# ProgramerSalar/stable-diffusion-from-scratch

Hardware: AMD Instinct MI355X
Metric: images/sec (512×512, 50-step DDIM) at 1/2/4/8 MI355X; UNet step ms (higher is better)
Workload: dtype f16; 1 GPU; sd1-txt2img-512-ddim50; global_batch=16, batch_per_gpu=16, ddim_steps=50, parallelism=dp1

## Files before the change

include/sdk_amd.h:

```cpp
#ifndef SDK_AMD_H
#define SDK_AMD_H

#include <stdint.h>

#ifdef __cplusplus
extern "C" {
#endif

typedef void* sdk_stream_t;

enum sdk_status {
  SDK_OK = 0,
  SDK_EINVAL = -1,
  SDK_EHIP = -2,
  SDK_EWORKSPACE = -3
};

typedef struct {
  const void* src0;
  const void* src1;
  int32_t c_split;
  int32_t cin;
  int32_t ld0, ld1;
  int32_t h, w;
  int32_t ksize;
  int32_t stride, pad;
  int32_t upsample;
  const float* gn_scale;
  const float* gn_shift;
  int32_t silu;
  int32_t pad_end;
} sdk_conv_src;

enum sdk_out_mode {
  SDK_OUT_NHWC_F16 = 0,
  SDK_OUT_NCHW_F32 = 1,
  SDK_OUT_GEGLU_F16 = 2,
  SDK_OUT_ROWS_F32 = 3
};

typedef struct {
  int32_t batch, ho, wo, cout;
  int32_t nseg;
  sdk_conv_src seg[2];
  const void* weight;
  int32_t k_total;
  const float* bias;
  const float* row_bias;
  int32_t row_bias_ld;
  const void* residual;
  int32_t res_ld;
  void* out;
  int32_t out_ld;
  int32_t out_mode;
  int32_t split_k;
  float* workspace;
  int64_t workspace_bytes;
  int32_t variant_hint;
  int32_t act;
  float* gn_partial;
  int64_t weight_batch_stride;
  int32_t split_inlaunch;
  uint32_t* tile_counters;
  int32_t tile_group_m;
  int32_t upsample_phase;
} sdk_conv_args;

#define SDK_TILE_COUNTERS 16384

enum sdk_conv_act {
  SDK_ACT_NONE = 0,
  SDK_ACT_QUICK_GELU = 1,
  SDK_ACT_GELU = 2
};

typedef struct {
  int32_t split_k;
  int32_t grid_tiles;
  int64_t workspace_bytes;
  int32_t variant;
  double flops;
  int32_t gn_chunks;
} sdk_conv_plan_info;

int sdk_conv2d_plan(const sdk_conv_args* a, sdk_conv_plan_info* info);
int sdk_conv2d(const sdk_conv_args* a, sdk_stream_t stream);

typedef struct {
  const void* src0; const void* src1;
  int32_t c_split, ld0, ld1;
  int32_t batch, hw, channels, groups;
  float eps;
  const float* gamma; const float* beta;
  float* scale; float* shift;
  float* workspace; int64_t workspace_bytes;
} sdk_group_norm_args;

int64_t sdk_group_norm_workspace(int32_t batch, int32_t hw, int32_t channels);
int sdk_group_norm_affine(const sdk_group_norm_args* a, sdk_stream_t stream);

int sdk_group_norm_apply(const sdk_group_norm_args* a, int32_t silu, void* y, int32_t ld_y, sdk_stream_t stream);

int sdk_group_norm_apply_padded(const sdk_group_norm_args* a, int32_t silu, void* y, int32_t ld_y, int32_t h,
                                int32_t w, int32_t pad, sdk_stream_t stream);

int sdk_group_norm(const sdk_group_norm_args* a, int32_t silu, void* y, int32_t ld_y, int32_t h, int32_t w,
                   int32_t pad, const float* part0, int32_t nch0, const float* part1, int32_t nch1,
                   sdk_stream_t stream);

int sdk_group_norm_finalize(const sdk_group_norm_args* a, const float* part0, int32_t nch0, const float* part1,
                            int32_t nch1, sdk_stream_t stream);

int sdk_group_norm_apply_ex(const sdk_group_norm_args* a, int32_t silu, const float* post_bias, int32_t pb_ld,
                            const void* residual, int32_t res_ld, void* y, int32_t ld_y, sdk_stream_t stream);

enum { SDK_GN_STATS_GIVEN = 0,
       SDK_GN_STATS_SLICE,
       SDK_GN_STATS_CHUNKED,
       SDK_GN_STATS_PARTS };
enum { SDK_GN_APPLY_NONE = 0,
       SDK_GN_APPLY_IN_STATS,
       SDK_GN_APPLY_FLAT, SDK_GN_APPLY_ROW, SDK_GN_APPLY_STRIDE };
typedef struct { int32_t stats, apply, launches; int64_t workspace_bytes; } sdk_group_norm_plan_info;
int sdk_group_norm_plan(const sdk_group_norm_args* a, int32_t want_stats, int32_t want_apply, int32_t h, int32_t w,
                        int32_t pad, int32_t nch0, int32_t nch1, int32_t allow_single_launch,
                        sdk_group_norm_plan_info* info);

double sdk_probe_mfma_flops(int32_t m16, int32_t blocks, int32_t iters);
int sdk_probe_mfma(int32_t m16, int32_t blocks, int32_t iters, const void* seed, float* sink, sdk_stream_t stream);
int sdk_probe_copy(const void* src, void* dst, int64_t bytes, sdk_stream_t stream);
int sdk_probe_copy_ex(const void* src, void* dst, int64_t bytes, int32_t mode, sdk_stream_t stream);

int sdk_layer_norm(const void* x, void* y, int32_t rows, int32_t cols, int32_t ld_x, int32_t ld_y,
                   const float* gamma, const float* beta, float eps, sdk_stream_t stream);

typedef struct {
  const void* q; const void* k; const void* v; void* o;
  int32_t q_ld, k_ld, v_ld, o_ld;
  int32_t batch, heads, nq, nk, head_dim;
  float scale;
  int32_t causal;
} sdk_attention_args;

int sdk_attention(const sdk_attention_args* a, sdk_stream_t stream);

enum { SDK_ATTN_AUTO = 0, SDK_ATTN_NW4, SDK_ATTN_NW8, SDK_ATTN_NW8_STAG, SDK_ATTN_QB2, SDK_ATTN_WIDE };
#define SDK_ATTN_WIDE_ROWS 64
#define SDK_ATTN_WIDE_KT 32
typedef struct { int32_t form, dqk, dv, waves, qblocks, stagger, seed_col, causal, grid; } sdk_attention_form_info;
int sdk_attention_form(const sdk_attention_args* a, int32_t form, sdk_attention_form_info* ran ,
                       sdk_stream_t stream);

typedef struct {
  const void* q; const void* k; const void* v; void* o;
  int32_t q_ld, k_ld, v_ld, o_ld;
  int32_t batch, heads, n, dim_head;
  void* workspace; int64_t workspace_bytes;
} sdk_linear_attention_args;
int32_t sdk_linear_attention_chunks(int32_t n);
int64_t sdk_linear_attention_workspace_bytes(const sdk_linear_attention_args* a);
int sdk_linear_attention(const sdk_linear_attention_args* a, sdk_stream_t stream);

typedef struct {
  const void* t; const void* kv; const void* wq; const void* wo; const float* bias; const void* res;
  void* out;
  int32_t t_ld, kv_ld, w_ld, res_ld, out_ld;
  int32_t batch, n_img, nk, channels, head_dim;
  float scale;
} sdk_xattn_args;

int sdk_cross_attention_block_supported(int32_t channels, int32_t head_dim, int32_t nk, int32_t n_img);
int sdk_xattn_pack_weight(const void* w, int32_t w_ld, void* packed, int32_t channels, sdk_stream_t stream);
int sdk_cross_attention_block(const sdk_xattn_args* a, sdk_stream_t stream);

typedef struct {
  const float* in_gamma; const float* in_beta; float in_eps;
  const float* out_gamma; const float* out_beta; float out_eps;
  void* out_ln; int32_t out_ln_ld;
} sdk_xattn_ln_args;

int sdk_cross_attention_block_ln(const sdk_xattn_args* a, const sdk_xattn_ln_args* ln, sdk_stream_t stream);

int sdk_segment_softmax(const float* s, int32_t ld_s, void* p, int32_t ld_p, int32_t rows, int32_t nseg,
                        int32_t seglen, float scale, sdk_stream_t stream);

typedef struct {
  const void* t; const void* res; void* out; const void* packed; const float* b2;
  int32_t t_ld, res_ld, out_ld;
  int32_t rows, channels, features;
} sdk_ff_args;

int sdk_ff_supported(int32_t channels, int32_t features);
int64_t sdk_ff_packed_bytes(int32_t channels, int32_t features);
int sdk_ff_pack(const void* w1, const float* b1, const void* w2, void* packed, int32_t channels, int32_t features,
                sdk_stream_t stream);
int sdk_feed_forward(const sdk_ff_args* a, sdk_stream_t stream);

typedef struct {
  const void* x; const void* w; const float* bias; const void* res; void* out;
  int32_t x_ld, res_ld, out_ld;
  int32_t rows, in_features, out_features;
} sdk_token_linear_args;

int sdk_token_linear_supported(int32_t in_features, int32_t out_features);
int sdk_token_linear(const sdk_token_linear_args* a, sdk_stream_t stream);

int sdk_token_linear_ln(const sdk_token_linear_args* a, const float* gamma, const float* beta, float eps,
                        void* out_ln, int32_t out_ln_ld, sdk_stream_t stream);

typedef struct {
  const float* x; const float* e; const float* e_uncond; const float* noise;
  float* x_prev; float* pred_x0;
  int64_t n;
  float sqrt_one_minus_at, sqrt_at, dir_coef, sqrt_a_prev, sigma, temperature;
  float guidance;
  int32_t v_param;
  float v_sqrt_a, v_sqrt_1ma;
} sdk_ddim_args;

int sdk_ddim_step(const sdk_ddim_args* a, sdk_stream_t stream);

int sdk_ddim_xprev(const sdk_ddim_args* a, sdk_stream_t stream);

typedef struct {
  const float* x; const float* model_out; const float* noise; const float* x_recon_in;
  float* x_prev; float* x_recon;
  int64_t n;
  int32_t stage, x0_param, clip;
  float c_recip, c_recipm1, coef1, coef2, sigma, nonzero, temperature;
} sdk_posterior_args;

int sdk_posterior_step(const sdk_posterior_args* a, sdk_stream_t stream);

typedef struct {
  const float* x0; const float* noise; const float* mask; const float* img;
  float* out;
  int64_t n, per_sample;
  int32_t hw, mask_mode;
  float sqrt_acp, sqrt_1m_acp;
} sdk_masked_q_args;

int sdk_masked_q_sample(const sdk_masked_q_args* a, sdk_stream_t stream);

int sdk_cfg_combine(const float* e_uncond, const float* e_cond, float* out, int64_t n, float guidance,
                    sdk_stream_t stream);

typedef struct {
  sdk_ddim_args step;
  int32_t pred_x0_in;
  float drop_scale;
  const uint8_t* keep;
  sdk_masked_q_args blend;
} sdk_ddim_ex_args;

int sdk_ddim_step_ex(const sdk_ddim_ex_args* a, sdk_stream_t stream);

typedef struct {
  sdk_posterior_args step;
  const uint8_t* keep;
  float drop_scale;
} sdk_posterior_ex_args;

int sdk_posterior_step_ex(const sdk_posterior_ex_args* a, sdk_stream_t stream);

enum { SDK_MULTISTEP_PLMS = 0, SDK_MULTISTEP_PLMS_WARMUP = 1, SDK_MULTISTEP_DPM = 2 };

typedef struct {
  sdk_ddim_args step;
  const float* hist[3];
  const float* e_next;
  float* hist_out;
  int32_t form, nhist;
  float c_x, c_0, c_1;
  int32_t reserved;
  sdk_masked_q_args blend;
} sdk_multistep_args;

int sdk_multistep_step(const sdk_multistep_args* a, sdk_stream_t stream);

typedef struct {
  const float* src[4];
  int32_t channels[4];
  int32_t nsrc;
  void* y;
  int32_t batch, hw, c_pad;
} sdk_concat_args;

int sdk_concat_nchw_to_nhwc(const sdk_concat_args* a, sdk_stream_t stream);

typedef struct {
  const float* src[4];
  int32_t channels[4];
  int32_t nsrc;
  void* y;
  int32_t batch, h, w, c_pad;
  int32_t kh, kw, sy, sx;
  int32_t p0, np;
} sdk_patch_pack_args;

int sdk_patch_pack(const sdk_patch_pack_args* a, sdk_stream_t stream);

int sdk_vq_code_norms(const float* codebook, float* norms, int32_t n, int32_t d, sdk_stream_t stream);

int32_t sdk_vq_nearest_splits(int64_t m, int32_t n, int32_t d);

int sdk_vq_nearest(const float* z, const float* codebook, const float* norms, int64_t* idx, float* z_q,
                   int32_t batch, int32_t d, int32_t hw, int32_t n, void* keys, int64_t keys_bytes,
                   int32_t force_splits, sdk_stream_t stream);

int sdk_vq_lookup(const int64_t* idx, const float* codebook, float* out, int64_t m, int32_t n, int32_t d,
                  int32_t hw, int32_t nchw, sdk_stream_t stream);

int sdk_vq_remap(const int64_t* inds, const int64_t* used, const int64_t* rnd, int64_t* out, int64_t count,
                 int32_t n_used, int32_t mode, int64_t unknown, int32_t extra, sdk_stream_t stream);

int sdk_ddpm_step(const float* x, const float* eps, const float* noise, float* out, int64_t n,
                  float inv_sqrt_alpha, float coef, float sigma, sdk_stream_t stream);

int sdk_timestep_embedding(const int64_t* t, const float* freqs, void* out, int32_t batch, int32_t dim,
                           sdk_stream_t stream);

int sdk_nchw_to_nhwc(const float* x, void* y, int32_t batch, int32_t channels, int32_t hw, int32_t c_pad,
                     float scale, sdk_stream_t stream);

int sdk_diag_gaussian_sample(const float* moments, const float* noise, float* z, int32_t batch, int32_t channels,
                             int32_t hw, float scale, sdk_stream_t stream);

int sdk_stochastic_encode(const float* x0, const float* noise, float* out, int64_t n, float sqrt_a,
                          float sqrt_1ma, sdk_stream_t stream);

int sdk_token_embedding(const int64_t* ids, const float* tok, const float* pos, void* out, int32_t batch,
                        int32_t seq, int32_t dim, sdk_stream_t stream);

int sdk_extract_patches(const float* z, float* out, int32_t batch, int32_t channels, int32_t h, int32_t w,
                        int32_t kh, int32_t kw, int32_t sy, int32_t sx, sdk_stream_t stream);
int sdk_fold_patches(const float* patches, const float* pix_w, const float* l_w, float* out, int32_t batch,
                     int32_t channels, int32_t h, int32_t w, int32_t ph, int32_t pw, int32_t sy, int32_t sx,
                     int32_t ly, int32_t lx, sdk_stream_t stream);

int sdk_upsample_bilinear2x(const void* x, void* y, int32_t batch, int32_t h, int32_t w, int32_t channels,
                            sdk_stream_t stream);
int sdk_gelu(const void* x, void* y, int64_t n, sdk_stream_t stream);

int sdk_upsample_nearest2x_padded(const void* x, int32_t ld_x, void* y, int32_t batch, int32_t h, int32_t w,
                                  int32_t channels, int32_t pad, sdk_stream_t stream);

int sdk_zero_border(const void* x, int32_t ld_x, void* y, int32_t batch, int32_t h, int32_t w, int32_t channels,
                    int32_t pad, sdk_stream_t stream);

int sdk_group_norm_film(const sdk_group_norm_args* a, const float* film, int32_t film_ld, int32_t film_off,
                        int32_t silu, void* y, int32_t ld_y, int32_t h, int32_t w, int32_t pad, const float* part0,
                        int32_t nch0, const float* part1, int32_t nch1, sdk_stream_t stream);

enum { SDK_RESAMPLE_AVGPOOL2 = 0, SDK_RESAMPLE_NEAREST2 = 1 };
int sdk_group_norm_resample(const sdk_group_norm_args* a, int32_t mode, int32_t silu, int32_t h, int32_t w,
                            int32_t pad, void* y_act, void* y_raw, sdk_stream_t stream);

int sdk_embedding_add(const void* emb, const float* table, const int64_t* ids, void* out, int32_t batch, int32_t dim,
                      int32_t n, sdk_stream_t stream);

int sdk_embedding_rows(const int64_t* ids, const float* table, void* out, int32_t n, int32_t dim,
                       sdk_stream_t stream);

enum { SDK_RESIZE_NEAREST = 0, SDK_RESIZE_BILINEAR = 1, SDK_RESIZE_BICUBIC = 2, SDK_RESIZE_AREA = 3 };
typedef struct {
  const float* x;
  float* y;
  int32_t planes, h, w, out_h, out_w, mode;
  double scale_h, scale_w;
} sdk_resize2d_args;

int sdk_resize2d(const sdk_resize2d_args* a, sdk_stream_t stream);

const char* sdk_last_error(void);
int sdk_version(void);
const char* sdk_kernel_name(int32_t variant);

#ifdef __cplusplus
}
#endif
#endif
```

stable-diffusion-from-scratch_amd/_lib.py:

```python
from __future__ import annotations

import ctypes as C
import os

_HERE = os.path.dirname(os.path.abspath(__file__))
LIB_PATH = os.environ.get("SD_AMD_LIB") or os.path.join(_HERE, "libsdk_amd.so")

vp = C.c_void_p
i32 = C.c_int32
i64 = C.c_int64
f32 = C.c_float
fp = C.POINTER(C.c_float)


class ConvSrc(C.Structure):
    _fields_ = [("src0", vp), ("src1", vp), ("c_split", i32), ("cin", i32), ("ld0", i32), ("ld1", i32),
                ("h", i32), ("w", i32), ("ksize", i32), ("stride", i32), ("pad", i32), ("upsample", i32),
                ("gn_scale", vp), ("gn_shift", vp), ("silu", i32), ("pad_end", i32)]


class ConvArgs(C.Structure):
    _fields_ = [("batch", i32), ("ho", i32), ("wo", i32), ("cout", i32), ("nseg", i32), ("seg", ConvSrc * 2),
                ("weight", vp), ("k_total", i32), ("bias", vp), ("row_bias", vp), ("row_bias_ld", i32),
                ("residual", vp), ("res_ld", i32), ("out", vp), ("out_ld", i32), ("out_mode", i32),
                ("split_k", i32), ("workspace", vp), ("workspace_bytes", i64), ("variant_hint", i32),
                ("act", i32), ("gn_partial", vp), ("weight_batch_stride", i64), ("split_inlaunch", i32),
                ("tile_counters", vp), ("tile_group_m", i32), ("upsample_phase", i32)]


class ConvPlanInfo(C.Structure):
    _fields_ = [("split_k", i32), ("grid_tiles", i32), ("workspace_bytes", i64), ("variant", i32),
                ("flops", C.c_double), ("gn_chunks", i32)]


class GroupNormArgs(C.Structure):
    _fields_ = [("src0", vp), ("src1", vp), ("c_split", i32), ("ld0", i32), ("ld1", i32), ("batch", i32),
                ("hw", i32), ("channels", i32), ("groups", i32), ("eps", f32), ("gamma", vp), ("beta", vp),
                ("scale", vp), ("shift", vp), ("workspace", vp), ("workspace_bytes", i64)]


class GroupNormPlanInfo(C.Structure):
    _fields_ = [("stats", i32), ("apply", i32), ("launches", i32), ("workspace_bytes", i64)]


class AttentionArgs(C.Structure):
    _fields_ = [("q", vp), ("k", vp), ("v", vp), ("o", vp), ("q_ld", i32), ("k_ld", i32), ("v_ld", i32),
                ("o_ld", i32), ("batch", i32), ("heads", i32), ("nq", i32), ("nk", i32), ("head_dim", i32),
                ("scale", f32), ("causal", i32)]


class AttentionFormInfo(C.Structure):
    _fields_ = [("form", i32), ("dqk", i32), ("dv", i32), ("waves", i32), ("qblocks", i32), ("stagger", i32),
                ("seed_col", i32), ("causal", i32), ("grid", i32)]


class LinearAttentionArgs(C.Structure):
    _fields_ = [("q", vp), ("k", vp), ("v", vp), ("o", vp), ("q_ld", i32), ("k_ld", i32), ("v_ld", i32),
                ("o_ld", i32), ("batch", i32), ("heads", i32), ("n", i32), ("dim_head", i32), ("workspace", vp),
                ("workspace_bytes", i64)]


class XAttnArgs(C.Structure):
    _fields_ = [("t", vp), ("kv", vp), ("wq", vp), ("wo", vp), ("bias", vp), ("res", vp), ("out", vp),
                ("t_ld", i32), ("kv_ld", i32), ("w_ld", i32), ("res_ld", i32), ("out_ld", i32), ("batch", i32),
                ("n_img", i32), ("nk", i32), ("channels", i32), ("head_dim", i32), ("scale", f32)]


class XAttnLnArgs(C.Structure):
    _fields_ = [("in_gamma", vp), ("in_beta", vp), ("in_eps", f32), ("out_gamma", vp), ("out_beta", vp),
                ("out_eps", f32), ("out_ln", vp), ("out_ln_ld", i32)]


class FfArgs(C.Structure):
    _fields_ = [("t", vp), ("res", vp), ("out", vp), ("packed", vp), ("b2", vp), ("t_ld", i32), ("res_ld", i32),
                ("out_ld", i32), ("rows", i32), ("channels", i32), ("features", i32)]


class TokenLinearArgs(C.Structure):
    _fields_ = [("x", vp), ("w", vp), ("bias", vp), ("res", vp), ("out", vp), ("x_ld", i32), ("res_ld", i32),
                ("out_ld", i32), ("rows", i32), ("in_features", i32), ("out_features", i32)]


class DdimArgs(C.Structure):
    _fields_ = [("x", vp), ("e", vp), ("e_uncond", vp), ("noise", vp), ("x_prev", vp), ("pred_x0", vp),
                ("n", i64), ("sqrt_one_minus_at", f32), ("sqrt_at", f32), ("dir_coef", f32), ("sqrt_a_prev", f32),
                ("sigma", f32), ("temperature", f32), ("guidance", f32), ("v_param", i32), ("v_sqrt_a", f32),
                ("v_sqrt_1ma", f32)]


class PosteriorArgs(C.Structure):
    _fields_ = [("x", vp), ("model_out", vp), ("noise", vp), ("x_recon_in", vp), ("x_prev", vp), ("x_recon", vp),
                ("n", i64), ("stage", i32), ("x0_param", i32), ("clip", i32), ("c_recip", f32), ("c_recipm1", f32),
                ("coef1", f32), ("coef2", f32), ("sigma", f32), ("nonzero", f32), ("temperature", f32)]


class MaskedQArgs(C.Structure):
    _fields_ = [("x0", vp), ("noise", vp), ("mask", vp), ("img", vp), ("out", vp), ("n", i64), ("per_sample", i64),
                ("hw", i32), ("mask_mode", i32), ("sqrt_acp", f32), ("sqrt_1m_acp", f32)]


class DdimExArgs(C.Structure):
    _fields_ = [("step", DdimArgs), ("pred_x0_in", i32), ("drop_scale", f32), ("keep", vp), ("blend", MaskedQArgs)]


class MultistepArgs(C.Structure):
    _fields_ = [("step", DdimArgs), ("hist", vp * 3), ("e_next", vp), ("hist_out", vp), ("form", i32), ("nhist", i32),
                ("c_x", f32), ("c_0", f32), ("c_1", f32), ("reserved", i32), ("blend", MaskedQArgs)]


class PosteriorExArgs(C.Structure):
    _fields_ = [("step", PosteriorArgs), ("keep", vp), ("drop_scale", f32)]


class ConcatArgs(C.Structure):
    _fields_ = [("src", vp * 4), ("channels", i32 * 4), ("nsrc", i32), ("y", vp), ("batch", i32), ("hw", i32),
                ("c_pad", i32)]


class PatchPackArgs(C.Structure):
    _fields_ = [("src", vp * 4), ("channels", i32 * 4), ("nsrc", i32), ("y", vp), ("batch", i32), ("h", i32),
                ("w", i32), ("c_pad", i32), ("kh", i32), ("kw", i32), ("sy", i32), ("sx", i32), ("p0", i32),
                ("np", i32)]


class Resize2dArgs(C.Structure):
    _fields_ = [("x", vp), ("y", vp), ("planes", i32), ("h", i32), ("w", i32), ("out_h", i32), ("out_w", i32),
                ("mode", i32), ("scale_h", C.c_double), ("scale_w", C.c_double)]


OUT_NHWC_F16, OUT_NCHW_F32, OUT_GEGLU_F16, OUT_ROWS_F32 = 0, 1, 2, 3
RESIZE_NEAREST, RESIZE_BILINEAR, RESIZE_BICUBIC, RESIZE_AREA = range(4)
ACT_NONE, ACT_QUICK_GELU, ACT_GELU = 0, 1, 2
ATTN_AUTO, ATTN_NW4, ATTN_NW8, ATTN_NW8_STAG, ATTN_QB2, ATTN_WIDE = range(6)
MULTISTEP_PLMS, MULTISTEP_PLMS_WARMUP, MULTISTEP_DPM = range(3)
ATTN_WIDE_ROWS, ATTN_WIDE_KT = 64, 32
RESAMPLE_AVGPOOL2, RESAMPLE_NEAREST2 = 0, 1
GN_STATS = ("given", "slice", "chunked", "parts")
GN_APPLY = ("none", "in_stats", "flat", "row", "stride")

EXPORTS = ["sdk_conv2d_plan", "sdk_conv2d", "sdk_group_norm_workspace", "sdk_group_norm_affine", "sdk_group_norm_apply", "sdk_group_norm_apply_padded", "sdk_group_norm_apply_ex", "sdk_group_norm", "sdk_group_norm_finalize", "sdk_group_norm_plan", "sdk_layer_norm",
           "sdk_attention", "sdk_attention_form", "sdk_linear_attention", "sdk_linear_attention_workspace_bytes", "sdk_linear_attention_chunks", "sdk_cross_attention_block_supported", "sdk_xattn_pack_weight", "sdk_cross_attention_block", "sdk_cross_attention_block_ln", "sdk_segment_softmax", "sdk_ff_supported", "sdk_ff_packed_bytes", "sdk_ff_pack", "sdk_feed_forward", "sdk_token_linear_supported", "sdk_token_linear", "sdk_token_linear_ln", "sdk_ddim_step", "sdk_ddim_xprev", "sdk_ddim_step_ex", "sdk_multistep_step", "sdk_cfg_combine", "sdk_posterior_step", "sdk_posterior_step_ex", "sdk_masked_q_sample", "sdk_concat_nchw_to_nhwc", "sdk_patch_pack", "sdk_ddpm_step", "sdk_timestep_embedding", "sdk_nchw_to_nhwc",
           "sdk_diag_gaussian_sample", "sdk_stochastic_encode", "sdk_token_embedding", "sdk_extract_patches",
           "sdk_fold_patches", "sdk_vq_code_norms", "sdk_vq_nearest_splits", "sdk_vq_nearest", "sdk_vq_lookup", "sdk_vq_remap",
           "sdk_upsample_bilinear2x", "sdk_upsample_nearest2x_padded", "sdk_zero_border", "sdk_gelu",
           "sdk_group_norm_film", "sdk_group_norm_resample", "sdk_embedding_add", "sdk_embedding_rows", "sdk_resize2d", "sdk_last_error", "sdk_version", "sdk_kernel_name",
           "sdk_probe_mfma_flops", "sdk_probe_mfma", "sdk_probe_copy", "sdk_probe_copy_ex"]

_lib = None


def lib():
    global _lib
    if _lib is not None:
        return _lib
    if not os.path.exists(LIB_PATH):
        raise RuntimeError(f"sd_amd: HIP library not built ({LIB_PATH} missing); run __graft_entry__.build()")
    import torch
    L = C.CDLL(LIB_PATH)
    L.sdk_conv2d_plan.argtypes = [C.POINTER(ConvArgs), C.POINTER(ConvPlanInfo)]
    L.sdk_conv2d.argtypes = [C.POINTER(ConvArgs), vp]
    L.sdk_group_norm_workspace.argtypes = [i32, i32, i32]
    L.sdk_group_norm_workspace.restype = i64
    L.sdk_group_norm_affine.argtypes = [C.POINTER(GroupNormArgs), vp]
    L.sdk_group_norm_apply.argtypes = [C.POINTER(GroupNormArgs), i32, vp, i32, vp]
    L.sdk_group_norm_apply_padded.argtypes = [C.POINTER(GroupNormArgs), i32, vp, i32, i32, i32, i32, vp]
    L.sdk_group_norm_apply_ex.argtypes = [C.POINTER(GroupNormArgs), i32, vp, i32, vp, i32, vp, i32, vp]
    L.sdk_group_norm.argtypes = [C.POINTER(GroupNormArgs), i32, vp, i32, i32, i32, i32, vp, i32, vp, i32, vp]
    L.sdk_group_norm_finalize.argtypes = [C.POINTER(GroupNormArgs), vp, i32, vp, i32, vp]
    L.sdk_group_norm_film.argtypes = [C.POINTER(GroupNormArgs), vp, i32, i32, i32, vp, i32, i32, i32, i32, vp, i32, vp,
                                      i32, vp]
    L.sdk_group_norm_plan.argtypes = [C.POINTER(GroupNormArgs), i32, i32, i32, i32, i32, i32, i32, i32,
                                      C.POINTER(GroupNormPlanInfo)]
    L.sdk_group_norm_resample.argtypes = [C.POINTER(GroupNormArgs), i32, i32, i32, i32, i32, vp, vp, vp]
    L.sdk_embedding_add.argtypes = [vp, vp, vp, vp, i32, i32, i32, vp]
    L.sdk_embedding_rows.argtypes = [vp, vp, vp, i32, i32, vp]
    L.sdk_resize2d.argtypes = [C.POINTER(Resize2dArgs), vp]
    L.sdk_upsample_bilinear2x.argtypes = [vp, vp, i32, i32, i32, i32, vp]
    L.sdk_upsample_nearest2x_padded.argtypes = [vp, i32, vp, i32, i32, i32, i32, i32, vp]
    L.sdk_zero_border.argtypes = [vp, i32, vp, i32, i32, i32, i32, i32, vp]
    L.sdk_gelu.argtypes = [vp, vp, i64, vp]
    L.sdk_layer_norm.argtypes = [vp, vp, i32, i32, i32, i32, vp, vp, f32, vp]
    L.sdk_attention.argtypes = [C.POINTER(AttentionArgs), vp]
    L.sdk_attention_form.argtypes = [C.POINTER(AttentionArgs), i32, C.POINTER(AttentionFormInfo), vp]
    L.sdk_linear_attention.argtypes = [C.POINTER(LinearAttentionArgs), vp]
    L.sdk_linear_attention_workspace_bytes.argtypes = [C.POINTER(LinearAttentionArgs)]
    L.sdk_linear_attention_workspace_bytes.restype = i64
    L.sdk_linear_attention_chunks.argtypes = [i32]
    L.sdk_linear_attention_chunks.restype = i32
    L.sdk_cross_attention_block_supported.argtypes = [i32, i32, i32, i32]
    L.sdk_xattn_pack_weight.argtypes = [vp, i32, vp, i32, vp]
    L.sdk_cross_attention_block.argtypes = [C.POINTER(XAttnArgs), vp]
    L.sdk_cross_attention_block_ln.argtypes = [C.POINTER(XAttnArgs), C.POINTER(XAttnLnArgs), vp]
    L.sdk_segment_softmax.argtypes = [vp, i32, vp, i32, i32, i32, i32, f32, vp]
    L.sdk_ff_supported.argtypes = [i32, i32]
    L.sdk_ff_packed_bytes.argtypes = [i32, i32]
    L.sdk_ff_packed_bytes.restype = i64
    L.sdk_ff_pack.argtypes = [vp, vp, vp, vp, i32, i32, vp]
    L.sdk_feed_forward.argtypes = [C.POINTER(FfArgs), vp]
    L.sdk_token_linear_supported.argtypes = [i32, i32]
    L.sdk_token_linear.argtypes = [C.POINTER(TokenLinearArgs), vp]
    L.sdk_token_linear_ln.argtypes = [C.POINTER(TokenLinearArgs), vp, vp, f32, vp, i32, vp]
    L.sdk_ddim_step.argtypes = [C.POINTER(DdimArgs), vp]
    L.sdk_ddim_xprev.argtypes = [C.POINTER(DdimArgs), vp]
    L.sdk_posterior_step.argtypes = [C.POINTER(PosteriorArgs), vp]
    L.sdk_ddim_step_ex.argtypes = [C.POINTER(DdimExArgs), vp]
    L.sdk_multistep_step.argtypes = [C.POINTER(MultistepArgs), vp]
    L.sdk_cfg_combine.argtypes = [vp, vp, vp, i64, f32, vp]
    L.sdk_posterior_step_ex.argtypes = [C.POINTER(PosteriorExArgs), vp]
    L.sdk_masked_q_sample.argtypes = [C.POINTER(MaskedQArgs), vp]
    L.sdk_concat_nchw_to_nhwc.argtypes = [C.POINTER(ConcatArgs), vp]
    L.sdk_patch_pack.argtypes = [C.POINTER(PatchPackArgs), vp]
    L.sdk_vq_code_norms.argtypes = [vp, vp, i32, i32, vp]
    L.sdk_vq_nearest_splits.argtypes = [i64, i32, i32]
    L.sdk_vq_nearest_splits.restype = i32
    L.sdk_vq_nearest.argtypes = [vp, vp, vp, vp, vp, i32, i32, i32, i32, vp, i64, i32, vp]
    L.sdk_vq_lookup.argtypes = [vp, vp, vp, i64, i32, i32, i32, i32, vp]
    L.sdk_vq_remap.argtypes = [vp, vp, vp, vp, i64, i32, i32, i64, i32, vp]
    L.sdk_ddpm_step.argtypes = [vp, vp, vp, vp, i64, f32, f32, f32, vp]
    L.sdk_timestep_embedding.argtypes = [vp, vp, vp, i32, i32, vp]
    L.sdk_nchw_to_nhwc.argtypes = [vp, vp, i32, i32, i32, i32, f32, vp]
    L.sdk_diag_gaussian_sample.argtypes = [vp, vp, vp, i32, i32, i32, f32, vp]
    L.sdk_stochastic_encode.argtypes = [vp, vp, vp, i64, f32, f32, vp]
    L.sdk_token_embedding.argtypes = [vp, vp, vp, vp, i32, i32, i32, vp]
    L.sdk_extract_patches.argtypes = [vp, vp, i32, i32, i32, i32, i32, i32, i32, i32, vp]
    L.sdk_fold_patches.argtypes = [vp, vp, vp, vp, i32, i32, i32, i32, i32, i32, i32, i32, i32, i32, vp]
    L.sdk_probe_mfma_flops.argtypes = [i32, i32, i32]
    L.sdk_probe_mfma_flops.restype = C.c_double
    L.sdk_probe_mfma.argtypes = [i32, i32, i32, vp, vp, vp]
    L.sdk_probe_copy.argtypes = [vp, vp, i64, vp]
    L.sdk_probe_copy_ex.argtypes = [vp, vp, i64, i32, vp]
    L.sdk_last_error.restype = C.c_char_p
    L.sdk_kernel_name.restype = C.c_char_p
    L.sdk_kernel_name.argtypes = [i32]
    for name in EXPORTS:
        if not hasattr(L, name):
            raise RuntimeError(f"sd_amd: {LIB_PATH} does not export {name}")
    _lib = L
    return L


def check(rc: int, what: str):
    if rc != 0:
        msg = lib().sdk_last_error().decode(errors="replace")
        raise RuntimeError(f"sd_amd.{what} failed ({rc}): {msg}")
```

stable-diffusion-from-scratch_amd/build.py:

```python
from __future__ import annotations

import concurrent.futures as cf
import os
import re
import subprocess

HERE = os.path.dirname(os.path.abspath(__file__))
CSRC = os.path.join(HERE, "csrc")
BUILD = os.path.join(HERE, "build")
LIB = os.path.join(HERE, "libsdk_amd.so")
SOURCES = ["norm.hip", "attention.hip", "attention_wide.hip", "linattn.hip", "sampler.hip", "xattn.hip", "ff.hip", "token.hip", "vq.hip", "cond.hip", "probe.hip"]
CONV_TILE_PARTS = 5


def _units():
    yield "conv_plan.hip", "conv_plan", []
    yield "conv_small.hip", "conv_small", []
    yield "conv_rowpanel.hip", "conv_rowpanel", []
    for k in range(1, CONV_TILE_PARTS + 1):
        yield "conv_tile.hip", f"conv_tile_p{k}", [f"-DSDK_CONV_PART={k}"]
    for src in SOURCES:
        yield src, src.replace(".hip", ""), []


def _deps(src: str, csrc: str):
    headers = [os.path.join(csrc, "common.h"), os.path.join(HERE, "..", "include", "sdk_amd.h")]
    if src.startswith("conv"):
        headers += sorted(os.path.join(csrc, f) for f in os.listdir(csrc) if f.startswith("conv") and f.endswith(".h"))
    return [os.path.join(csrc, src)] + headers
HIPCC = os.environ.get("HIPCC", "/opt/rocm/bin/hipcc")
FLAGS = ["--offload-arch=gfx950", "-O3", "-fPIC", "-std=c++17", "-Wno-unused-result"]
EXTRA = {"attention.hip": ["-mno-amdgpu-ieee", "-fno-honor-nans"],
         "attention_wide.hip": ["-mno-amdgpu-ieee", "-fno-honor-nans"]}
REMARK = "-Rpass-analysis=kernel-resource-usage"
NO_SCRATCH = re.compile(r"token_linear320_kernel|attn_wide_kernel|conv_rowpanel_kernel")
WARN_SCRATCH = re.compile(r"conv_glds_kernel|conv_ph_kernel|ff_geglu_kernel|xattn_block_kernel|attn_fwd_kernel|vq_nearest_")
_RES = re.compile(r"remark: (?:Function Name: (\S+)|\s+(VGPRs|AGPRs|ScratchSize \[bytes/lane\]|Occupancy \[waves/SIMD\]): (\d+))")


def resource_usage(stderr: str):
    out = []
    for m in _RES.finditer(stderr):
        if m.group(1):
            out.append((m.group(1), {}))
        elif out:
            out[-1][1][m.group(2).split(" ")[0]] = int(m.group(3))
    return out


def _needs(obj: str, deps) -> bool:
    if not os.path.exists(obj):
        return True
    t = os.path.getmtime(obj)
    return any(os.path.getmtime(d) > t for d in deps)


def build(force: bool = False, verbose: bool = False, diag: bool = False, tag: str = "", defines=(),
          extra=None, csrc: str = CSRC) -> str:
    suffix = "_diag" if diag else (f"_{tag}" if tag else "")
    bdir = BUILD + suffix
    lib = LIB.replace(".so", f"{suffix}.so")
    extra_flags = dict(EXTRA)
    for k, v in (extra or {}).items():
        extra_flags[k] = extra_flags.get(k, []) + list(v)
    os.makedirs(bdir, exist_ok=True)
    jobs = []
    objs = []
    for src, stem, udefs in _units():
        s = os.path.join(csrc, src)
        o = os.path.join(bdir, stem + ".o")
        objs.append(o)
        flags_file = o + ".flags"
        dflags = (["-DSDK_CONV_DIAGNOSTICS"] if diag else []) + list(defines) + udefs
        fl = " ".join(FLAGS + extra_flags.get(src, []) + dflags)
        stale_flags = not os.path.exists(flags_file) or open(flags_file).read() != fl
        if force or stale_flags or _needs(o, _deps(src, csrc)) or not os.path.exists(o + ".res"):
            for stale in (o, flags_file):
                if os.path.exists(stale):
                    os.remove(stale)
            jobs.append(([HIPCC, *FLAGS, *dflags, *extra_flags.get(src, []), REMARK, "-c", s, "-o", o],
                         (flags_file, fl)))

    def run(cmd, sidecar=None):
        r = subprocess.run(cmd, capture_output=True, text=True)
        if r.returncode != 0:
            raise RuntimeError(f"hipcc failed: {' '.join(cmd)}\n{r.stdout}\n{r.stderr}")
        if REMARK in cmd:
            usage = resource_usage(r.stderr)
            obj = cmd[cmd.index("-o") + 1]
            with open(obj + ".res", "w") as f:
                for name, u in usage:
                    f.write(f"{name} vgpr={u.get('VGPRs')} agpr={u.get('AGPRs')} scratch={u.get('ScratchSize')} "
                            f"occ={u.get('Occupancy')}\n")
            if os.path.basename(obj).startswith("token") and not any(
                    NO_SCRATCH.search(n) and "ScratchSize" in u for n, u in usage):
                os.remove(obj)
                raise RuntimeError("no kernel-resource-usage remark for token_linear320_kernel: cannot verify "
                                   "that it uses no scratch")
            bad = [n for n, u in usage if NO_SCRATCH.search(n) and u.get("ScratchSize", 0) > 0]
            for n, u in usage:
                if WARN_SCRATCH.search(n) and u.get("ScratchSize", 0) > 0:
                    print(f"warning: {n} uses {u['ScratchSize']} B/lane of scratch", flush=True)
            if bad:
                os.remove(obj)
                raise RuntimeError("counted-vmcnt kernels use scratch (spills break the hand-counted waits): " +
                                   ", ".join(bad))
        if sidecar:
            with open(sidecar[0], "w") as f:
                f.write(sidecar[1])
        if verbose:
            print(" ".join(cmd))
        return r

    workers = int(os.environ.get("SD_AMD_BUILD_JOBS", "8"))
    with cf.ThreadPoolExecutor(max_workers=min(workers, max(1, len(jobs)))) as ex:
        list(ex.map(lambda j: run(*j), jobs))
    if force or jobs or _needs(lib, objs):
        run([HIPCC, "--offload-arch=gfx950", "-shared", "-fPIC", *objs, "-o", lib])
        with open(os.path.join(bdir, "resource_usage.txt"), "w") as f:
            for o in objs:
                if os.path.exists(o + ".res"):
                    f.write(open(o + ".res").read())
    return lib


if __name__ == "__main__":
    import sys
    print(build(verbose=True, diag="--diag" in sys.argv))
```

stable-diffusion-from-scratch_amd/csrc/common.h:

```cpp
#pragma once
#include <hip/hip_runtime.h>
#include <stdint.h>

#include <atomic>
#include <string>

#include "../../include/sdk_amd.h"

namespace sdk {

typedef _Float16 half_t;
typedef _Float16 h8 __attribute__((ext_vector_type(8)));
typedef _Float16 h4 __attribute__((ext_vector_type(4)));
typedef _Float16 h2 __attribute__((ext_vector_type(2)));
typedef float f16v __attribute__((ext_vector_type(16)));
typedef float f4 __attribute__((ext_vector_type(4)));
typedef float f2 __attribute__((ext_vector_type(2)));

void set_error(const std::string& msg);
int fail(int code, const std::string& msg);
int check_launch(const char* what);
int attention_wide(const sdk_attention_args* a, hipStream_t s, sdk_attention_form_info* ran);

inline int ensure_dyn_lds(const void* fn, int bytes, std::atomic<unsigned long long>& done, const char* what) {
  int dev = 0;
  if (hipGetDevice(&dev) != hipSuccess) return fail(SDK_EHIP, std::string(what) + ": hipGetDevice failed");
  const unsigned long long bit = 1ull << (dev & 63);
  if (done.load(std::memory_order_acquire) & bit) return SDK_OK;
  if (hipFuncSetAttribute(fn, hipFuncAttributeMaxDynamicSharedMemorySize, bytes) != hipSuccess)
    return fail(SDK_EHIP, std::string(what) + ": cannot raise the dynamic LDS limit");
  done.fetch_or(bit, std::memory_order_acq_rel);
  return SDK_OK;
}

__device__ __forceinline__ float silu_f(float x) { return x / (1.0f + __expf(-x)); }
__device__ __forceinline__ float erf_fast(float x) {
  const float a = fabsf(x);
  const float t = __builtin_amdgcn_rcpf(fmaf(0.3275911f, a, 1.0f));
  float y = fmaf(1.061405429f, t, -1.453152027f);
  y = fmaf(y, t, 1.421413741f);
  y = fmaf(y, t, -0.284496736f);
  y = fmaf(y, t, 0.254829592f);
  y *= t;
  const float r = 1.0f - y * __expf(-a * a);
  return copysignf(r, x);
}
__device__ __forceinline__ float gelu_erf(float x) { return 0.5f * x * (1.0f + erf_fast(x * 0.70710678118654752f)); }

__device__ __forceinline__ int xcd_remap(int bid, int nblk) {
  const int q = nblk >> 3, r = nblk & 7, x = bid & 7, i = bid >> 3;
  return (x < r ? x * (q + 1) : r * (q + 1) + (x - r) * q) + i;
}

#ifndef SDK_XLANE_DPP
#define SDK_XLANE_DPP 0
#endif
template <int CTRL>
__device__ __forceinline__ float dpp_f(float x) {
  static_assert(CTRL <= 0xFF || CTRL == 0x124 || CTRL == 0x128, "dpp_f: quad_perm, row_ror:4 or row_ror:8");
#if SDK_XLANE_DPP
  return __builtin_bit_cast(float, __builtin_amdgcn_update_dpp(0, __builtin_bit_cast(int, x), CTRL, 0xF, 0xF, false));
#else
  constexpr int pat = CTRL <= 0xFF ? 0x8000 | CTRL : (0x1F | ((CTRL == 0x124 ? 4 : 8) << 10));
  return __builtin_bit_cast(float, __builtin_amdgcn_ds_swizzle(__builtin_bit_cast(int, x), pat));
#endif
}
__device__ __forceinline__ float readlane_f(float x, int l) {
  return __builtin_bit_cast(float, __builtin_amdgcn_readlane(__builtin_bit_cast(int, x), l));
}
__device__ __forceinline__ float wave_sum_f(float x) {
  x += dpp_f<0xB1>(x);
  x += dpp_f<0x4E>(x);
  x += dpp_f<0x124>(x);
  x += dpp_f<0x128>(x);
  return (readlane_f(x, 0) + readlane_f(x, 16)) + (readlane_f(x, 32) + readlane_f(x, 48));
}

template <int MAXV>
__device__ __forceinline__ void ln_row_stats(const h8 (&v)[MAXV], int cols, float eps, float& mean, float& rstd) {
#pragma clang fp contract(off)
  const int lane = threadIdx.x & 63;
  const int c8 = cols / 8;
  const float x0 = readlane_f((float)v[0][0], 0);
  float s1 = 0.f, s2 = 0.f;
#pragma unroll
  for (int i = 0; i < MAXV; ++i) {
    const bool ok = lane + 64 * i < c8;
#pragma unroll
    for (int j = 0; j < 8; ++j) {
      const float d = ok ? (float)v[i][j] - x0 : 0.f;
      s1 += d;
      s2 = __builtin_fmaf(d, d, s2);
    }
  }
  s1 = wave_sum_f(s1);
  s2 = wave_sum_f(s2);
  const float inv_n = 1.f / cols;
  const float dm = s1 * inv_n;
  const float var = fmaxf(__builtin_fmaf(-dm, dm, s2 * inv_n), 0.f);
  mean = x0 + dm;
  rstd = rsqrtf(var + eps);
}

template <int CPL>
__device__ __forceinline__ void ln_quad_stats(const h8 (&v)[CPL], float eps, float& mean, float& rstd) {
#pragma clang fp contract(off)
  const float x0 = dpp_f<0x00>((float)v[0][0]);
  float s1 = 0.f, s2 = 0.f;
#pragma unroll
  for (int i = 0; i < CPL; ++i)
#pragma unroll
    for (int j = 0; j < 8; ++j) {
      const float d = (float)v[i][j] - x0;
      s1 += d;
      s2 = __builtin_fmaf(d, d, s2);
    }
  s1 += dpp_f<0xB1>(s1);
  s2 += dpp_f<0xB1>(s2);
  s1 += dpp_f<0x4E>(s1);
  s2 += dpp_f<0x4E>(s2);
  const float inv_n = 1.f / (32 * CPL);
  const float dm = s1 * inv_n;
  const float var = fmaxf(__builtin_fmaf(-dm, dm, s2 * inv_n), 0.f);
  mean = x0 + dm;
  rstd = rsqrtf(var + eps);
}

__device__ __forceinline__ h8 ln_quad_apply(const h8& v, float mean, float rstd, const float* gb, int C, int k) {
#pragma clang fp contract(off)
  const f4 g0 = *reinterpret_cast<const f4*>(gb + 8 * k), g1 = *reinterpret_cast<const f4*>(gb + 8 * k + 4);
  const f4 b0 = *reinterpret_cast<const f4*>(gb + C + 8 * k), b1 = *reinterpret_cast<const f4*>(gb + C + 8 * k + 4);
  h8 o;
#pragma unroll
  for (int j = 0; j < 4; ++j) {
    o[j] = (half_t)__builtin_fmaf(((float)v[j] - mean) * rstd, g0[j], b0[j]);
    o[4 + j] = (half_t)__builtin_fmaf(((float)v[4 + j] - mean) * rstd, g1[j], b1[j]);
  }
  return o;
}

__device__ __forceinline__ h8 ln_apply8(const h8& v, float mean, float rstd, const float (&g)[8], const float (&b)[8]) {
#pragma clang fp contract(off)
  h8 o;
#pragma unroll
  for (int j = 0; j < 8; ++j) o[j] = (half_t)__builtin_fmaf(((float)v[j] - mean) * rstd, g[j], b[j]);
  return o;
}

}
```

stable-diffusion-from-scratch_amd/csrc/norm.hip:

```cpp
#include <algorithm>
#include <string>

#include "common.h"

namespace sdk {
namespace {

constexpr int GN_U = 8;

struct GnGeom {
  int c8, nv, ry, chunk_rows, nchunks;
};

GnGeom gn_geom(int batch, int hw, int channels) {
  GnGeom g;
  g.c8 = channels / 8;
  g.nv = (g.c8 + 255) / 256;
  g.ry = g.nv > 1 ? 1 : std::max(1, 256 / g.c8);
  const int step = g.ry * GN_U;
  const int want = std::max(1, (1536 + batch - 1) / std::max(batch, 1));
  const int per = std::max(1, (hw + want - 1) / want);
  g.chunk_rows = (per + step - 1) / step * step;
  g.nchunks = (hw + g.chunk_rows - 1) / g.chunk_rows;
  return g;
}

__device__ __forceinline__ h8 load_px(const half_t* s0, const half_t* s1, int c_split, int ld0, int ld1,
                                      size_t pix, int c) {
  if (c < c_split) return *reinterpret_cast<const h8*>(s0 + pix * ld0 + c);
  return *reinterpret_cast<const h8*>(s1 + pix * ld1 + (c - c_split));
}

__device__ __forceinline__ void gn_load8(const float* p, float o[8]) {
  const f4* q = reinterpret_cast<const f4*>(p);
  const f4 a = q[0], b = q[1];
#pragma unroll
  for (int j = 0; j < 4; ++j) { o[j] = a[j]; o[4 + j] = b[j]; }
}

__device__ __forceinline__ float gn_act(float x, float sc, float sh, int silu) {
  float t = x * sc + sh;
  if (silu) t = t * __builtin_amdgcn_rcpf(1.0f + __expf(-t));
  return t;
}

__device__ __forceinline__ h8 gn_act8(h8 v, const float sc[8], const float sh[8], int silu) {
  h8 o;
#pragma unroll
  for (int j = 0; j < 8; ++j) o[j] = (half_t)gn_act((float)v[j], sc[j], sh[j], silu);
  return o;
}

__global__ void __launch_bounds__(256) gn_partial_kernel(const half_t* s0, const half_t* s1, int c_split, int ld0,
                                                         int ld1, int hw, int channels, GnGeom g, float2* partial) {
  extern __shared__ __attribute__((aligned(16))) float red[];
  const int tid = threadIdx.x, chunk = blockIdx.x, b = blockIdx.y;
  const int r0 = chunk * g.chunk_rows, r1 = min(hw, r0 + g.chunk_rows);
  const size_t img = (size_t)b * hw;
  const int ysub = tid / g.c8;
  for (int vi = 0; vi < g.nv; ++vi) {
    const int vec = g.nv > 1 ? tid + vi * 256 : tid % g.c8;
    const bool active = vec < g.c8 && ysub < g.ry;
    float sum[8], sq[8], piv[8];
#pragma unroll
    for (int j = 0; j < 8; ++j) { sum[j] = 0.f; sq[j] = 0.f; piv[j] = 0.f; }
    if (active) {
      const int c = vec * 8;
      const h8 pv = load_px(s0, s1, c_split, ld0, ld1, img, c);
#pragma unroll
      for (int j = 0; j < 8; ++j) piv[j] = (float)pv[j];
      const int rstart = r0 + (g.nv > 1 ? 0 : ysub);
      const int rstep = g.nv > 1 ? 1 : g.ry;
      for (int r = rstart; r < r1; r += GN_U * rstep) {
        h8 v[GN_U];
#pragma unroll
        for (int u = 0; u < GN_U; ++u) {
          const int rr = r + u * rstep;
          v[u] = rr < r1 ? load_px(s0, s1, c_split, ld0, ld1, img + rr, c) : pv;
        }
#pragma unroll
        for (int u = 0; u < GN_U; ++u)
#pragma unroll
          for (int j = 0; j < 8; ++j) {
            const float d = (float)v[u][j] - piv[j];
            sum[j] += d;
            sq[j] += d * d;
          }
      }
    }
    if (g.ry == 1) {
      if (active) {
#pragma unroll
        for (int j = 0; j < 8; ++j)
          partial[((size_t)b * g.nchunks + chunk) * channels + vec * 8 + j] = make_float2(sum[j], sq[j]);
      }
      continue;
    }
    const int C = g.c8 * 8;
    if (active) {
#pragma unroll
      for (int j = 0; j < 8; ++j) {
        red[ysub * C + vec * 8 + j] = sum[j];
        red[(g.ry + ysub) * C + vec * 8 + j] = sq[j];
      }
    }
    __syncthreads();
    for (int c = tid; c < C; c += 256) {
      float a = 0.f, q = 0.f;
      for (int y = 0; y < g.ry; ++y) { a += red[y * C + c]; q += red[(g.ry + y) * C + c]; }
      partial[((size_t)b * g.nchunks + chunk) * channels + c] = make_float2(a, q);
    }
  }
}

__device__ __forceinline__ double wave_sum_d(double v) {
  for (int off = 32; off > 0; off >>= 1) v += __shfl_xor(v, off, 64);
  return v;
}

__global__ void __launch_bounds__(256) gn_finalize_kernel(const half_t* s0, const half_t* s1, int c_split, int ld0,
                                                          int ld1, int hw, int channels, int groups, GnGeom g,
                                                          const float2* partial, float eps, const float* gamma,
                                                          const float* beta, float* scale, float* shift) {
  __shared__ double cm[256], cq[256];
  const int grp = blockIdx.x, b = blockIdx.y, tid = threadIdx.x, lane = tid & 63, wave = tid >> 6;
  const int cg = channels / groups, c0 = grp * cg;
  const size_t img = (size_t)b * hw;
  const double n = (double)hw;
  int tpc = 64;
  while (tpc > 1 && tpc * cg > 256) tpc >>= 1;
  const int ci = tid / tpc, sub = tid - ci * tpc;
  for (int cbase = 0; cbase < cg; cbase += 256 / tpc) {
    const int cc = cbase + ci;
    const bool act = ci < 256 / tpc && cc < cg;
    double a1 = 0.0, a2 = 0.0;
    if (act) {
      const float2* pp = partial + (size_t)b * g.nchunks * channels + c0 + cc;
      for (int k = sub; k < g.nchunks; k += tpc) {
        const float2 v = pp[(size_t)k * channels];
        a1 += v.x;
        a2 += v.y;
      }
    }
    for (int off = tpc >> 1; off > 0; off >>= 1) {
      a1 += __shfl_xor(a1, off, 64);
      a2 += __shfl_xor(a2, off, 64);
    }
    if (act && sub == 0) {
      const int c = c0 + cc;
      const float piv = c < c_split ? (float)s0[img * ld0 + c] : (float)s1[img * ld1 + (c - c_split)];
      cm[cc] = (double)piv + a1 / n;
      cq[cc] = a2 - a1 * a1 / n;
    }
  }
  __syncthreads();
  if (wave != 0) return;
  double mean_sum = 0.0, m2_sum = 0.0, msq_sum = 0.0;
  for (int ci = lane; ci < cg; ci += 64) {
    mean_sum += cm[ci];
    msq_sum += cm[ci] * cm[ci];
    m2_sum += cq[ci];
  }
  mean_sum = wave_sum_d(mean_sum);
  msq_sum = wave_sum_d(msq_sum);
  m2_sum = wave_sum_d(m2_sum);
  const double mg = mean_sum / cg;
  double m2g = m2_sum + n * (msq_sum - cg * mg * mg);
  if (m2g < 0) m2g = 0;
  const double var = m2g / (n * cg);
  const float rstd = (float)(1.0 / sqrt(var + (double)eps));
  const float meanf = (float)mg;
  for (int ci = lane; ci < cg; ci += 64) {
    const int c = c0 + ci;
    const float gm = gamma ? gamma[c] : 1.f, bt = beta ? beta[c] : 0.f;
    const float sc = gm * rstd;
    scale[(size_t)b * channels + c] = sc;
    shift[(size_t)b * channels + c] = bt - meanf * sc;
  }
}

constexpr int GNF_T = 512;
template <bool APPLY>
__global__ void __launch_bounds__(GNF_T) gn_stats_fused_kernel(const half_t* s0, const half_t* s1, int c_split,
                                                               int ld0, int ld1, int hw, int channels, int cg,
                                                               int gps, float eps, const float* gamma,
                                                               const float* beta, float* scale, float* shift,
                                                               int silu, half_t* y, int ldy, int h, int w, int pad) {
  __shared__ float2 red[GNF_T * 8];
  __shared__ double cmean[512], cm2[512];
  const int tid = threadIdx.x, b = blockIdx.y;
  const int sc = gps * cg, c0 = blockIdx.x * sc;
  const int cv = sc / 8, rp = GNF_T / cv;
  const int v = tid % cv, r0 = tid / cv;
  const bool active = r0 < rp;
  const size_t img = (size_t)b * hw;
  const int c = c0 + 8 * v;
  float sum[8], sq[8], piv[8];
#pragma unroll
  for (int j = 0; j < 8; ++j) { sum[j] = 0.f; sq[j] = 0.f; piv[j] = 0.f; }
  if (active) {
    const h8 pv = load_px(s0, s1, c_split, ld0, ld1, img, c);
#pragma unroll
    for (int j = 0; j < 8; ++j) piv[j] = (float)pv[j];
    constexpr int U = 8;
    for (int r = r0; r < hw; r += U * rp) {
      h8 x[U];
#pragma unroll
      for (int u = 0; u < U; ++u) {
        const int rr = r + u * rp;
        x[u] = rr < hw ? load_px(s0, s1, c_split, ld0, ld1, img + rr, c) : pv;
      }
#pragma unroll
      for (int u = 0; u < U; ++u)
#pragma unroll
        for (int j = 0; j < 8; ++j) {
          const float d = (float)x[u][j] - piv[j];
          sum[j] += d;
          sq[j] += d * d;
        }
    }
#pragma unroll
    for (int j = 0; j < 8; ++j) red[r0 * sc + 8 * v + j] = make_float2(sum[j], sq[j]);
  }
  __syncthreads();
  const double n = (double)hw;
  for (int k = tid; k < sc; k += GNF_T) {
    double a1 = 0.0, a2 = 0.0;
    for (int r = 0; r < rp; ++r) {
      const float2 q = red[r * sc + k];
      a1 += q.x;
      a2 += q.y;
    }
    const int cc = c0 + k;
    const float p0 = cc < c_split ? (float)s0[img * ld0 + cc] : (float)s1[img * ld1 + (cc - c_split)];
    cmean[k] = (double)p0 + a1 / n;
    cm2[k] = a2 - a1 * a1 / n;
  }
  __syncthreads();
  for (int g = tid; g < gps; g += GNF_T) {
    double ms = 0.0, m2 = 0.0;
    for (int k = 0; k < cg; ++k) ms += cmean[g * cg + k];
    const double mg = ms / cg;
    for (int k = 0; k < cg; ++k) {
      const double dm = cmean[g * cg + k] - mg;
      m2 += cm2[g * cg + k] + n * dm * dm;
    }
    const double var = (m2 > 0 ? m2 : 0.0) / (n * cg);
    cmean[g * cg] = mg;
    cm2[g * cg] = 1.0 / sqrt(var + (double)eps);
  }
  __syncthreads();
  for (int k = tid; k < sc; k += GNF_T) {
    const int g = k / cg, cc = c0 + k;
    const float rstd = (float)cm2[g * cg], meanf = (float)cmean[g * cg];
    const float gm = gamma ? gamma[cc] : 1.f, bt = beta ? beta[cc] : 0.f;
    const float s = gm * rstd;
    if constexpr (APPLY) {
      red[k] = make_float2(s, bt - meanf * s);
    } else {
      scale[(size_t)b * channels + cc] = s;
      shift[(size_t)b * channels + cc] = bt - meanf * s;
    }
  }
  if constexpr (APPLY) {
    __syncthreads();
    if (!active) return;
    float sa[8], sh[8];
#pragma unroll
    for (int j = 0; j < 8; ++j) {
      const float2 t = red[8 * v + j];
      sa[j] = t.x;
      sh[j] = t.y;
    }
    const int wp = w + 2 * pad, npix = (h + 2 * pad) * wp;
    half_t* yb = y + (size_t)b * npix * ldy + c;
    constexpr int U = 4;
    for (int r = r0; r < npix; r += U * rp) {
      h8 x[U];
      bool in[U];
#pragma unroll
      for (int u = 0; u < U; ++u) {
        const int rr = r + u * rp;
        const int py = rr / wp - pad, px = rr - (rr / wp) * wp - pad;
        in[u] = rr < npix && (unsigned)py < (unsigned)h && (unsigned)px < (unsigned)w;
        x[u] = in[u] ? load_px(s0, s1, c_split, ld0, ld1, img + (size_t)py * w + px, c) : h8{};
      }
#pragma unroll
      for (int u = 0; u < U; ++u) {
        const int rr = r + u * rp;
        if (rr >= npix) continue;
        h8 o = {};
        if (in[u]) o = gn_act8(x[u], sa, sh, silu);
        *reinterpret_cast<h8*>(yb + (size_t)rr * ldy) = o;
      }
    }
  }
}

template <class Put>
__device__ __forceinline__ void gn_merge_group(const double* cm, const double* cq, int cg, double n, float eps, int c0,
                                               const float* gamma, const float* beta, int lane, Put put) {
  double mean_sum = 0.0;
  for (int ci = lane; ci < cg; ci += 64) mean_sum += cm[ci];
  mean_sum = wave_sum_d(mean_sum);
  const double mg = mean_sum / cg;
  double m2g = 0.0;
  for (int ci = lane; ci < cg; ci += 64) {
    const double dm = cm[ci] - mg;
    m2g += cq[ci] + n * dm * dm;
  }
  m2g = wave_sum_d(m2g);
  const double var = (m2g > 0 ? m2g : 0.0) / (n * cg);
  const float rstd = (float)(1.0 / sqrt(var + (double)eps));
  const float meanf = (float)mg;
  for (int ci = lane; ci < cg; ci += 64) {
    const int c = c0 + ci;
    const float gm = gamma ? gamma[c] : 1.f, bt = beta ? beta[c] : 0.f;
    const float sc = gm * rstd;
    put(ci, c, sc, bt - meanf * sc);
  }
}

__global__ void __launch_bounds__(256) gn_finalize_part_kernel(const float2* part0, int nch0, const float2* part1,
                                                               int nch1, int c_split, int hw, int channels,
                                                               int groups, float eps, const float* gamma,
                                                               const float* beta, float* scale, float* shift) {
  __shared__ double cm[256], cq[256];
  const int grp = blockIdx.x, b = blockIdx.y, tid = threadIdx.x, lane = tid & 63, wave = tid >> 6;
  const int cg = channels / groups, c0 = grp * cg;
  int tpc = 64;
  while (tpc > 1 && tpc * cg > 256) tpc >>= 1;
  const int ci = tid / tpc, sub = tid - ci * tpc;
  for (int cbase = 0; cbase < cg; cbase += 256 / tpc) {
    const int cc = cbase + ci;
    const bool act = ci < 256 / tpc && cc < cg;
    double mean = 0.0, m2 = 0.0, n = 0.0;
    if (act) {
      const int c = c0 + cc;
      const bool second = c >= c_split;
      const float2* pp = second ? part1 : part0;
      const int nch = second ? nch1 : nch0, cs = second ? channels - c_split : c_split, cl = second ? c - c_split : c;
      const double rows = (double)hw / nch;
      for (int k = sub; k < nch; k += tpc) {
        const float2 q = pp[((size_t)b * nch + k) * cs + cl];
        const double dl = (double)q.x - mean, nn = n + rows, f = rows / nn;
        mean += dl * f;
// ... 907 lines not shown
```

stable-diffusion-from-scratch_amd/openai_model/attention.py:

```python
from __future__ import annotations

import os
import math

import torch
from torch import nn

from .. import ops
from ..packing import f32, gn_norm, prep_norm
from .utils import conv_nd, normalization, zero_module


def Normalize(in_channels):
    return torch.nn.GroupNorm(num_groups=32, num_channels=in_channels, eps=1e-6, affine=True)


_FUSED_ENV = os.environ.get("SD_AMD_FUSED_XATTN")
FUSED_CROSS_ATTENTION = _FUSED_ENV != "0"
FUSED_XATTN_MIN_ROWS = 0 if _FUSED_ENV == "1" else 65536
FUSED_XATTN_640_MAX_ROWS = 16384
FUSED_XATTN_NORMS = os.environ.get("SD_AMD_XATTN_NORMS") != "0"


def _use_fused_xattn(channels, head_dim, nk, n_img, batch):
    if not FUSED_CROSS_ATTENTION or n_img % 64:
        return False
    rows = batch * n_img
    if _FUSED_ENV != "1":
        if channels == 320:
            if rows < FUSED_XATTN_MIN_ROWS:
                return False
        elif channels != 640 or rows > FUSED_XATTN_640_MAX_ROWS:
            return False
    return ops.cross_attention_block_supported(channels, head_dim, nk, n_img)


XATTN_REASSOC = os.environ.get("SD_AMD_XATTN_REASSOC") != "0"

FUSED_FF = os.environ.get("SD_AMD_FUSED_FF") != "0"
TOKEN_LINEAR = os.environ.get("SD_AMD_TOKEN_LINEAR", "1") != "0"


class ReassocContext:
    __slots__ = ("kv", "w1", "w2", "heads", "nk", "batch", "_build")

    def __init__(self, kv, heads, nk, batch, build):
        self.kv, self.heads, self.nk, self.batch, self._build = kv, heads, nk, batch, build
        self.w1 = self.w2 = None

    def weights(self):
        if self.w1 is None:
            if torch.cuda.is_available() and torch.cuda.is_current_stream_capturing():
                raise RuntimeError("ReassocContext: per-prompt weights are built eagerly — run one eager "
                                   "step with this context before capturing a graph")
            self.w1, self.w2 = self._build()
            self._build = None
        return self.w1, self.w2


def reassoc_weights(k, v, wq, wo):
    B, L, H, d = k.shape
    w1 = torch.einsum("bjhe,hec->bhjc", k, wq.view(H, d, -1)).reshape(B, H * L, -1)
    w2 = torch.einsum("che,bjhe->bchj", wo.view(wo.shape[0], H, d), v).reshape(B, wo.shape[0], H * L)
    return w1, w2


def _reassoc_applies(inner, heads, nk):
    kr = (heads * nk + ops.BK - 1) // ops.BK * ops.BK
    return XATTN_REASSOC and 2 * kr <= inner


class CrossAttention(nn.Module):

    def __init__(self, query_dim, context_dim=None, heads=8, dim_head=64, dropout=0.):
        super().__init__()
        inner_dim = dim_head * heads
        self.self_attn = context_dim is None
        context_dim = query_dim if context_dim is None else context_dim
        self.scale = dim_head ** -0.5
        self.heads = heads
        self.dim_head = dim_head
        self.to_q = nn.Linear(query_dim, inner_dim, bias=False)
        self.to_k = nn.Linear(context_dim, inner_dim, bias=False)
        self.to_v = nn.Linear(context_dim, inner_dim, bias=False)
        self.to_out = nn.Sequential(nn.Linear(inner_dim, query_dim), nn.Dropout(dropout))

    def _prepare(self, dev):
        qd = self.to_q.in_features
        cd = self.to_k.in_features
        if self.self_attn:
            w = torch.cat([self.to_q.weight, self.to_k.weight, self.to_v.weight], 0)
            self._pc_qkv = ops.PackedConv([(w, qd)], None, device=dev)
        self._pc_q = ops.PackedConv([(self.to_q.weight, qd)], None, device=dev)
        self._pc_kv = ops.PackedConv([(torch.cat([self.to_k.weight, self.to_v.weight], 0), cd)], None, device=dev)
        self._pc_o = ops.PackedConv([(self.to_out[0].weight, self.heads * self.dim_head)], self.to_out[0].bias,
                                    device=dev)
        inner = self.heads * self.dim_head
        self._ptl_o = (ops.PackedTokenLinear(self.to_out[0].weight, self.to_out[0].bias, dev)
                       if self.self_attn and ops.token_linear_supported(inner, self.to_out[0].out_features) else None)
        if not self.self_attn:
            self._bo32 = f32(self.to_out[0].bias, dev)
            self._pc_reassoc = None

    def context_kv(self, ctx2d, L=None):
        kv = ops.linear(self._pc_kv, ctx2d)
        inner = self.heads * self.dim_head
        if L is None or self.self_attn or not _reassoc_applies(inner, self.heads, L):
            return kv
        B, H, d = ctx2d.shape[0] // L, self.heads, self.dim_head
        C = self.to_q.in_features
        Co = self.to_out[0].out_features

        def build():
            dev = kv.device
            if self._pc_reassoc is None:
                wq, wo = self.to_q.weight.detach(), self.to_out[0].weight.detach()
                self._pc_reassoc = (
                    [ops.PackedConv([(wq[h * d:(h + 1) * d].t().contiguous(), d)], None, device=dev) for h in range(H)],
                    [ops.PackedConv([(wo[:, h * d:(h + 1) * d].contiguous(), d)], None, device=dev) for h in range(H)])
            pq, po = self._pc_reassoc
            kr = (H * L + ops.BK - 1) // ops.BK * ops.BK
            w1 = torch.zeros(B, (kr + ops.BN - 1) // ops.BN * ops.BN, C, dtype=torch.float16, device=dev)
            w2 = torch.zeros(B, (Co + ops.BN - 1) // ops.BN * ops.BN, kr, dtype=torch.float16, device=dev)
            w1h = w1[:, :H * L].view(B, H, L, C)
            for h in range(H):
                w1h[:, h] = ops.linear(pq[h], kv[:, h * d:(h + 1) * d]).view(B, L, C)
                w2[:, :Co, h * L:(h + 1) * L] = ops.linear(po[h], kv[:, inner + h * d:inner + (h + 1) * d]).view(
                    B, L, Co).transpose(1, 2)
            return ops.PerImageWeights(w1, H * L), ops.PerImageWeights(w2, Co, self._bo32)
        return ReassocContext(kv, H, L, B, build)

    def _run(self, t, residual, B, N, kv=None, Lc=None):
        inner = self.heads * self.dim_head
        if kv is None:
            if self.self_attn:
                qkv = ops.linear(self._pc_qkv, t)
                q, k, v, nk = qkv[:, :inner], qkv[:, inner:2 * inner], qkv[:, 2 * inner:], N
            else:
                q = ops.linear(self._pc_q, t)
                kvx = ops.linear(self._pc_kv, t)
                k, v, nk = kvx[:, :inner], kvx[:, inner:], N
        else:
            ops.PROFILER.region = "cross_attention"
            if isinstance(kv, ReassocContext):
                if t.stride(-1) == 1 and N % 128 == 0 and kv.batch == B:
                    w1, w2 = kv.weights()
                    s = ops.linear(w1, t, out_mode=ops.OUT_ROWS_F32, n_img=N)
                    p = ops.segment_softmax(s, kv.heads, kv.nk, self.scale, ld_p=w2.k_total)
                    out = ops.linear(w2, p, residual=residual, n_img=N)
                    ops.PROFILER.region = None
                    return out
                kv = kv.kv
            if t.stride(-1) == 1 and _use_fused_xattn(inner, self.dim_head, Lc, N, B):
                out = ops.cross_attention_block(t, kv, self._pc_q, self._pc_o, batch=B, n_img=N, nk=Lc,
                                                heads=self.heads, head_dim=self.dim_head, scale=self.scale,
                                                residual=residual)
                ops.PROFILER.region = None
                return out
            q = ops.linear(self._pc_q, t)
            k, v, nk = kv[:, :inner], kv[:, inner:], Lc
        o = ops.attention(q, k, v, batch=B, heads=self.heads, nq=N, nk=nk, head_dim=self.dim_head, scale=self.scale)
        if TOKEN_LINEAR and self._ptl_o is not None and o.stride(-1) == 1 and \
                (residual is None or residual.is_contiguous()):
            out = ops.token_linear(self._ptl_o, o, residual=residual)
        else:
            out = ops.linear(self._pc_o, o, residual=residual)
        ops.PROFILER.region = None
        return out


class GELU(nn.Module):

    def __init__(self, dim_in, dim_out):
        super().__init__()
        self.proj = nn.Linear(dim_in, dim_out * 2)


class FeedForward(nn.Module):

    def __init__(self, dim, dim_out=None, mult=4, glu=False, dropout=0.):
        super().__init__()
        inner_dim = int(dim * mult)
        dim_out = dim if dim_out is None else dim_out
        if not glu:
            raise NotImplementedError("sd_amd: only the gated (GEGLU) feed-forward is on the SD path")
        self.net = nn.Sequential(GELU(dim, inner_dim), nn.Dropout(dropout), nn.Linear(inner_dim, dim_out))

    def _prepare(self, dev):
        p = self.net[0].proj
        self._pc1 = ops.PackedConv([(p.weight, p.in_features)], p.bias, geglu=True, device=dev)
        self._pc2 = ops.PackedConv([(self.net[2].weight, self.net[2].in_features)], self.net[2].bias, device=dev)
        self._pff = None
        if FUSED_FF and ops.ff_supported(p.in_features, p.out_features // 2):
            self._pff = ops.PackedFF(p.weight, p.bias, self.net[2].weight, self.net[2].bias, dev)

    def _run(self, t, residual):
        if self._pff is not None and t.stride(-1) == 1:
            return ops.feed_forward(self._pff, t, residual=residual)
        g = ops.linear(self._pc1, t, out_mode=ops.OUT_GEGLU_F16)
        return ops.linear(self._pc2, g, residual=residual)


class BasicTransformerBlock(nn.Module):

    def __init__(self, dim, n_heads, d_head, dropout=0., context_dim=None, gated_ff=True, checkpoint=True):
        super().__init__()
        self.attn1 = CrossAttention(query_dim=dim, heads=n_heads, dim_head=d_head, dropout=dropout)
        self.ff = FeedForward(dim=dim, dropout=dropout, glu=gated_ff)
        self.attn2 = CrossAttention(query_dim=dim, context_dim=context_dim, heads=n_heads, dim_head=d_head,
                                    dropout=dropout)
        self.norm1 = nn.LayerNorm(dim)
        self.norm2 = nn.LayerNorm(dim)
        self.norm3 = nn.LayerNorm(dim)
        self.checkpoint = checkpoint

    def _prepare(self, dev):
        for m in (self.attn1, self.attn2, self.ff):
            m._prepare(dev)
        for n in (self.norm1, self.norm2, self.norm3):
            prep_norm(n, dev)

    def _run(self, tok, B, N, kv=None, Lc=None, t=None):
        if t is None:
            t = ops.layer_norm(tok, self.norm1._g, self.norm1._b, self.norm1.eps)
        tok = self.attn1._run(t, tok, B, N)
        a2 = self.attn2
        if (kv is not None and FUSED_XATTN_NORMS and tok.stride(-1) == 1
                and _use_fused_xattn(a2.heads * a2.dim_head, a2.dim_head, Lc, N, B)):
            ops.PROFILER.region = "cross_attention"
            tok, t = ops.cross_attention_block(
                tok, kv, a2._pc_q, a2._pc_o, batch=B, n_img=N, nk=Lc, heads=a2.heads, head_dim=a2.dim_head,
                scale=a2.scale, residual=tok, norm_in=(self.norm2._g, self.norm2._b, self.norm2.eps),
                norm_out=(self.norm3._g, self.norm3._b, self.norm3.eps))
            ops.PROFILER.region = None
            return self.ff._run(t, tok)
        t = ops.layer_norm(tok, self.norm2._g, self.norm2._b, self.norm2.eps)
        tok = self.attn2._run(t, tok, B, N, kv, Lc)
        t = ops.layer_norm(tok, self.norm3._g, self.norm3._b, self.norm3.eps)
        return self.ff._run(t, tok)


class SpatialTransformer(nn.Module):

    def __init__(self, in_channels, n_heads, d_head, depth=1, dropout=0., context_dim=None, use_linear=False):
        super().__init__()
        self.in_channels = in_channels
        inner_dim = n_heads * d_head
        self.inner_dim = inner_dim
        self.use_linear = use_linear
        self.norm = Normalize(in_channels)
        if use_linear:
            self.proj_in = nn.Linear(in_channels, inner_dim)
        else:
            self.proj_in = nn.Conv2d(in_channels, inner_dim, kernel_size=1, stride=1, padding=0)
        self.transformer_blocks = nn.ModuleList(
            [BasicTransformerBlock(inner_dim, n_heads, d_head, dropout=dropout, context_dim=context_dim)
             for _ in range(depth)])
        if use_linear:
            self.proj_out = zero_module(nn.Linear(in_channels, inner_dim))
        else:
            self.proj_out = zero_module(nn.Conv2d(inner_dim, in_channels, kernel_size=1, stride=1, padding=0))

    def _prepare(self, dev):
        prep_norm(self.norm, dev)
        self._pc_in = ops.PackedConv([(self.proj_in.weight, self.in_channels)], self.proj_in.bias, device=dev)
        self._ptl_in = (ops.PackedTokenLinear(self.proj_in.weight, self.proj_in.bias, dev)
                        if ops.token_linear_supported(self.in_channels, self.inner_dim) else None)
        self._pc_out = ops.PackedConv([(self.proj_out.weight, self.inner_dim)], self.proj_out.bias, device=dev)
        for blk in self.transformer_blocks:
            blk._prepare(dev)

    def context_kv(self, ctx2d, L=None):
        return [blk.attn2.context_kv(ctx2d, L) for blk in self.transformer_blocks]

    def _run(self, x, kvs=None, Lc=None):
        B, H, W, Cc = x.shape
        xn = gn_norm(self.norm, x, silu=False)
        t1 = None
        if TOKEN_LINEAR and self._ptl_in is not None and xn.is_contiguous():
            n1 = self.transformer_blocks[0].norm1 if len(self.transformer_blocks) else None
            if n1 is not None:
                tok, t1 = ops.token_linear(self._ptl_in, xn.view(B * H * W, Cc), norm=(n1._g, n1._b, n1.eps))
            else:
                tok = ops.token_linear(self._ptl_in, xn.view(B * H * W, Cc))
        else:
            tok = ops.conv2d(self._pc_in, xn).view(B * H * W, self.inner_dim)
        for i, blk in enumerate(self.transformer_blocks):
            tok = blk._run(tok, B, H * W, None if kvs is None else kvs[i], Lc, t=t1 if i == 0 else None)
        return ops.conv2d(self._pc_out, tok.view(B, H, W, self.inner_dim), residual=x, gn_stats=True)


class QKVAttentionLegacy(nn.Module):

    def __init__(self, n_heads):
        super().__init__()
        self.n_heads = n_heads

    def scale(self, ch):
        return 1.0 / math.sqrt(math.sqrt(ch))


class FlashAttention(nn.Module):

    def __init__(self, n_heads):
        super().__init__()
        self.n_heads = n_heads

    def scale(self, ch):
        return 1.0 / math.sqrt(ch)


class AttentionBlock(nn.Module):

    def __init__(self, channels, num_heads=1, num_head_channels=-1, use_checkpoint=False,
                 use_new_attention_order=False):
        super().__init__()
        self.channels = channels
        if num_head_channels == -1:
            self.num_heads = num_heads
        else:
            assert channels % num_head_channels == 0
            self.num_heads = channels // num_head_channels
        self.use_checkpoint = use_checkpoint
        self.norm = normalization(channels)
        self.qkv = conv_nd(1, channels, channels * 3, 1)
        self.attention = FlashAttention(self.num_heads) if use_new_attention_order else \
            QKVAttentionLegacy(self.num_heads)
        self.proj_out = zero_module(conv_nd(1, channels, channels, 1))

    def _prepare(self, dev):
        self.norm._prepare(dev)
        self._pc_qkv = ops.PackedConv([(self.qkv.weight, self.channels)], self.qkv.bias, device=dev)
        self._pc_proj = ops.PackedConv([(self.proj_out.weight, self.channels)], self.proj_out.bias, device=dev)

    def _run(self, x):
        B, H, W, Cc = x.shape
        xn = self.norm.norm(x, silu=False)
        qkv = ops.conv2d(self._pc_qkv, xn).view(B * H * W, 3 * Cc)
        ch = Cc // self.num_heads
        o = ops.attention(qkv[:, :Cc], qkv[:, Cc:2 * Cc], qkv[:, 2 * Cc:], batch=B, heads=self.num_heads,
                          nq=H * W, nk=H * W, head_dim=ch, scale=self.attention.scale(ch))
        return ops.conv2d(self._pc_proj, o.view(B, H, W, Cc), residual=x, gn_stats=True)
```

stable-diffusion-from-scratch_amd/ops.py:

```python
from __future__ import annotations

import ctypes as C
import math

import numpy as np
import torch

from . import _lib
from ._lib import (ACT_NONE, ACT_QUICK_GELU, ACT_GELU, AttentionArgs, XAttnArgs, XAttnLnArgs, FfArgs, TokenLinearArgs, ConvArgs, ConvPlanInfo, GroupNormArgs,
                   OUT_GEGLU_F16, OUT_NCHW_F32, OUT_NHWC_F16, OUT_ROWS_F32, check, lib)

BK = 64
BN = 128


def _stream():
    return C.c_void_p(torch.cuda.current_stream().cuda_stream)


def _ptr(t):
    return C.c_void_p(t.data_ptr()) if t is not None else None


def _need_cuda(t: torch.Tensor, what: str, dtype=torch.float16):
    if not isinstance(t, torch.Tensor) or not t.is_cuda:
        raise TypeError(f"sd_amd.{what}: expected a CUDA tensor (HIP path only, no CPU fallback)")
    if dtype is not None and t.dtype != dtype:
        raise TypeError(f"sd_amd.{what}: expected {dtype}, got {t.dtype}")


def need_gpu_sampler(option: str, device):
    if torch.device(device).type != "cuda":
        raise NotImplementedError(f"sd_amd: {option} is implemented on the GPU only (HIP kernels, no CPU "
                                  f"fallback); got device '{device}'")



class _Workspace:

    def __init__(self):
        self.buf = {}
        self.retired = []
        self.lane = 0

    def release_retired(self):
        self.retired.clear()

    def use_lane(self, lane: int):
        import contextlib

        @contextlib.contextmanager
        def cm():
            prev, self.lane = self.lane, lane
            try:
                yield
            finally:
                self.lane = prev
        return cm()

    def counters(self, device) -> torch.Tensor:
        key = (torch.device(device).index, self.lane, "cnt")
        c = self.buf.get(key)
        if c is None:
            if torch.cuda.is_current_stream_capturing():
                raise RuntimeError("sd_amd: tile counters must exist before graph capture (run one warm-up step)")
            c = torch.zeros(TILE_COUNTERS, dtype=torch.int32, device=device)
            self.buf[key] = c
        return c

    def get(self, nbytes: int, device) -> torch.Tensor:
        key = (torch.device(device).index, self.lane)
        b = self.buf.get(key)
        if b is None or b.numel() < nbytes:
            if torch.cuda.is_current_stream_capturing():
                raise RuntimeError("sd_amd: workspace must be sized before graph capture (run one warm-up step)")
            if b is not None:
                self.retired.append(b)
                nbytes = max(nbytes, 2 * b.numel())
            b = torch.empty(max(nbytes, 1 << 20), dtype=torch.uint8, device=device)
            self.buf[key] = b
        return b


WORKSPACE = _Workspace()
TILE_COUNTERS = 16384



def _as_pair(x):
    if isinstance(x, tuple):
        a, b = x
        return a, b
    return x, None


def src_shape(x):
    a, b = _as_pair(x)
    B, H, W, C0 = a.shape
    return B, H, W, C0 + (b.shape[-1] if b is not None else 0)


def _fill_src(s: "_lib.ConvSrc", x, ksize, stride, pad, upsample, gn, silu):
    a, b = _as_pair(x)
    _need_cuda(a, "conv2d")
    B, H, W, C0 = a.shape
    if a.stride(3) != 1 or (H > 1 and a.stride(1) != W * a.stride(2)) or (B > 1 and a.stride(0) != H * a.stride(1)):
        raise ValueError("sd_amd.conv2d: source must be NHWC with contiguous channels and a uniform pixel stride")
    s.src0 = a.data_ptr()
    s.ld0 = a.stride(2) if a.dim() == 4 else a.stride(1)
    if b is not None:
        _need_cuda(b, "conv2d")
        s.src1 = b.data_ptr()
        s.ld1 = b.stride(2)
        s.c_split = C0
        s.cin = C0 + b.shape[-1]
    else:
        s.src1 = None
        s.ld1 = 0
        s.c_split = C0
        s.cin = C0
    s.h, s.w = H, W
    s.ksize, s.stride, s.pad, s.upsample = ksize, stride, pad, 1 if upsample else 0
    if gn is not None:
        s.gn_scale, s.gn_shift = gn[0].data_ptr(), gn[1].data_ptr()
    else:
        s.gn_scale = s.gn_shift = None
    s.silu = 1 if silu else 0
    return B, H, W



class PackedConv:

    def __init__(self, segments, bias=None, geglu=False, device="cuda"):
        cols, self.seg_geom = [], []
        n_out = None
        for w, cin_src in segments:
            w = w.detach().float()
            if w.dim() == 2:
                w = w[:, :, None, None]
            if w.dim() == 3:
                w = w[:, :, :, None]
            N, Cin, kh, kw = w.shape
            assert kh == kw, "square kernels only"
            if n_out is None:
                n_out = N
            assert N == n_out
            cin_pad = (cin_src + BK - 1) // BK * BK
            wp = torch.zeros(N, kh, kw, cin_pad, dtype=torch.float32, device=w.device)
            wp[:, :, :, :Cin] = w.permute(0, 2, 3, 1)
            wp = wp.reshape(N, kh * kw, cin_pad // BK, BK).permute(0, 2, 1, 3)
            cols.append(wp.reshape(N, -1))
            self.seg_geom.append((kh, cin_src))
        Wt = torch.cat(cols, dim=1)
        b = bias.detach().float().clone() if bias is not None else None
        if geglu:
            inner = n_out // 2
            assert inner % 32 == 0
            idx = []
            for q in range(inner // 32):
                idx += list(range(32 * q, 32 * q + 32)) + list(range(inner + 32 * q, inner + 32 * q + 32))
            idx = torch.tensor(idx, device=Wt.device)
            Wt = Wt[idx]
            if b is not None:
                b = b[idx.to(b.device)]
        self.N = n_out
        self.geglu = geglu
        npad = (n_out + BN - 1) // BN * BN
        Wfull = torch.zeros(npad, Wt.shape[1], dtype=torch.float32, device=Wt.device)
        Wfull[:n_out] = Wt
        self.weight = Wfull.to(device=device, dtype=torch.float16).contiguous()
        self.k_total = self.weight.shape[1]
        self.bias = b.to(device=device, dtype=torch.float32).contiguous() if b is not None else None


class PerImageWeights:

    def __init__(self, weight, n, bias=None):
        assert weight.dim() == 3 and weight.dtype == torch.float16 and weight.is_contiguous()
        assert weight.shape[1] % BN == 0 and weight.shape[2] % BK == 0 and n <= weight.shape[1]
        self.weight = weight
        self.N = n
        self.k_total = weight.shape[2]
        self.bias = bias
        self.geglu = False
        self.seg_geom = [(1, weight.shape[2])]
        self.w_batch_stride = weight.shape[1] * weight.shape[2]


def fold_upsample_weight(w):
    assert w.dim() == 4 and w.shape[2:] == (3, 3)
    rows = ((w[:, :, 0], w[:, :, 1] + w[:, :, 2]), (w[:, :, 0] + w[:, :, 1], w[:, :, 2]))
    out = w.new_empty(4, w.shape[0], w.shape[1], 2, 2)
    for a in range(2):
        for dy in range(2):
            r = rows[a][dy]
            cols = ((r[:, :, 0], r[:, :, 1] + r[:, :, 2]), (r[:, :, 0] + r[:, :, 1], r[:, :, 2]))
            for b in range(2):
                for dx in range(2):
                    out[2 * a + b, :, :, dy, dx] = cols[b][dx]
    return out


class PhaseConv:

    def __init__(self, weight, cin_src, bias=None, device="cuda"):
        ph = fold_upsample_weight(weight.detach().float())
        packs = [PackedConv([(ph[q], cin_src)], bias if q == 0 else None, device=device) for q in range(4)]
        self.weight = torch.stack([pk.weight for pk in packs]).contiguous()
        self.N, self.k_total, self.bias = packs[0].N, packs[0].k_total, packs[0].bias
        self.geglu = False
        self.seg_geom = [(2, cin_src)]
        self.w_batch_stride = self.weight.shape[1] * self.weight.shape[2]


def _conv_source_files():
    import os
    src = os.environ.get("SD_AMD_CONV_SOURCE") or os.path.join(os.path.dirname(os.path.abspath(__file__)), "csrc")
    if not os.path.isdir(src):
        src = os.path.dirname(src)
    return [os.path.join(src, f) for f in sorted(os.listdir(src)) if f.startswith("conv")]


def _conv_source_hash():
    import hashlib
    import os
    h = hashlib.sha1()
    for path in _conv_source_files():
        h.update(os.path.basename(path).encode() + b"\0")
        with open(path, "rb") as f:
            h.update(f.read())
    return h.hexdigest()[:16]


class _Autotune:
    VARIANTS = (2, 7, 6, 4, 3, 8, 9, 16, 17, 18, 19, 20, 21, 22, 23, 24, 25, 26, 31, 32, 33, 34, 35, 38, 40, 49)
    SPLITS = (0, 1, 2, 3, 4, 6, 8, 12, 16, -2)
    GROUPS = (1, 8, 16)

    def __init__(self):
        import os
        self.enabled = False
        self.table = {}
        self.timed = 0
        ev = os.environ.get("SD_AMD_TUNE_VARIANTS")
        if ev:
            self.VARIANTS = tuple(int(v) for v in ev.split(","))
        self.reps = int(os.environ.get("SD_AMD_TUNE_REPS", "3"))

    def enable(self, on=True):
        self.enabled = on

    def save(self, path):
        import json
        with open(path, "w") as f:
            json.dump({"device": torch.cuda.get_device_name(0) if torch.cuda.is_available() else None,
                       "conv_source": _conv_source_hash(),
                       "entries": [[list(k), list(v)] for k, v in sorted(self.table.items(), key=str)]}, f, indent=0)

    def load(self, path):
        import json
        with open(path) as f:
            d = json.load(f)
        if d.get("conv_source") != _conv_source_hash():
            return 0
        n = 0
        for k, v in d["entries"]:
            self.table[tuple(k)] = tuple(v)
            n += 1
        return n

    def key(self, a, pc, gn=False):
        s0, s1 = a.seg[0], a.seg[1]
        return (a.batch, a.ho, a.wo, a.cout, a.nseg, pc.k_total, a.out_mode, s0.cin, s0.h, s0.w, s0.ksize,
                s0.stride, s0.upsample, s0.c_split, int(bool(s0.gn_scale) or bool(s0.silu)),
                s1.cin if a.nseg > 1 else 0, int(gn), int(bool(a.weight_batch_stride)))

    def choose(self, a, pc, dev, gn=False):
        key = self.key(a, pc, gn)
        hit = self.table.get(key)
        if hit is not None or not self.enabled or torch.cuda.is_current_stream_capturing():
            return hit
        cands = self.VARIANTS
        if a.nseg > 1 and (a.seg[1].gn_scale or a.seg[1].silu):
            self.table[key] = (0, 0)
            return self.table[key]
        if a.seg[0].gn_scale or a.seg[0].silu:
            cands = (0, 35)
        best, best_t = (0, 0), float("inf")
        info = ConvPlanInfo()
        stream = _stream()
        emit_any = False
        if gn:
            for v in cands:
                for sp in self.SPLITS:
                    a.variant_hint = v + 1
                    set_split(a, sp, dev)
                    if lib().sdk_conv2d_plan(C.byref(a), C.byref(info)) == 0 and info.gn_chunks > 0:
                        emit_any = True
        for v in cands:
            for sp in self.SPLITS:
                a.variant_hint = v + 1
                set_split(a, sp, dev)
                if lib().sdk_conv2d_plan(C.byref(a), C.byref(info)) != 0:
                    continue
                if info.variant != v:
                    continue
                if sp == 0 and info.split_k in self.SPLITS[1:]:
                    continue
                part = None
                if emit_any:
                    if info.gn_chunks == 0:
# ... 488 lines not shown
    B, Cc, H, W = x.shape
    Ho, Wo = math.floor(H * sh), math.floor(W * sw)
    if min(B, Cc, H, W, Ho, Wo) < 1:
        raise ValueError(f"sd_amd.resize2d: empty input or output ({tuple(x.shape)} -> {Ho} x {Wo})")
    if B * Cc >= 2 ** 31 or max(H, W, Ho, Wo) >= 2 ** 31:
        raise ValueError("sd_amd.resize2d: sizes exceed int32")
    x = x.contiguous()
    if out is None:
        out = torch.empty(B, Cc, Ho, Wo, dtype=torch.float32, device=x.device)
    else:
        _need_cuda(out, "resize2d out", torch.float32)
        if tuple(out.shape) != (B, Cc, Ho, Wo) or not out.is_contiguous() or out.device != x.device:
            raise ValueError(f"sd_amd.resize2d: out must be contiguous {(B, Cc, Ho, Wo)} on the input's device")
    a = _lib.Resize2dArgs()
    a.x, a.y = x.data_ptr(), out.data_ptr()
    a.planes, a.h, a.w, a.out_h, a.out_w = B * Cc, H, W, Ho, Wo
    a.mode, a.scale_h, a.scale_w = RESIZE_MODES[mode], sh, sw
    if PROFILER.active:
        PROFILER.begin("resize2d", None, nbytes=4 * (x.numel() + out.numel()))
    check(lib().sdk_resize2d(C.byref(a), _stream()), "resize2d")
    if PROFILER.active:
        PROFILER.end()
    return out


def layer_norm(x2d, gamma, beta, eps=1e-5, out=None):
    _need_cuda(x2d, "layer_norm")
    M, Cc = x2d.shape
    y = _claim(out) if out is not None else torch.empty(M, Cc, dtype=torch.float16, device=x2d.device)
    if PROFILER.active:
        PROFILER.begin("layer_norm", None)
    check(lib().sdk_layer_norm(_ptr(x2d), _ptr(y), M, Cc, x2d.stride(0), y.stride(0), _ptr(gamma), _ptr(beta),
                               C.c_float(eps), _stream()), "layer_norm")
    if PROFILER.active:
        PROFILER.end()
    return y



def probe_peaks(reps=3):
    dev = torch.device("cuda", torch.cuda.current_device())
    seed = torch.randn(32768, device=dev).half()
    nsm = torch.cuda.get_device_properties(dev).multi_processor_count
    sink = torch.empty(4 * nsm * 4, dtype=torch.float32, device=dev)
    out = {}
    for m16, iters, name in ((1, 40000, "mfma_16x16x32_f16_tflops"), (0, 20000, "mfma_32x32x16_f16_tflops")):
        top = 0.0
        for blocks in (2 * nsm, 4 * nsm):
            check(lib().sdk_probe_mfma(m16, blocks, 200, _ptr(seed), _ptr(sink), _stream()), "probe_mfma")
            best = float("inf")
            for _ in range(reps):
                e0, e1 = torch.cuda.Event(enable_timing=True), torch.cuda.Event(enable_timing=True)
                e0.record()
                check(lib().sdk_probe_mfma(m16, blocks, iters, _ptr(seed), _ptr(sink), _stream()), "probe_mfma")
                e1.record()
                e1.synchronize()
                best = min(best, e0.elapsed_time(e1))
            top = max(top, lib().sdk_probe_mfma_flops(m16, blocks, iters) / (best * 1e-3) / 1e12)
        out[name] = round(top, 1)
    nbytes = 1 << 30
    src = torch.empty(nbytes // 2, dtype=torch.float16, device=dev).normal_()
    dst = torch.empty_like(src)
    best_gbs, best_mode = 0.0, 0
    for mode in (0, 1, 2, 3, 1 | (8 << 2), 3 | (8 << 2), 1 | (32 << 2), 3 | (32 << 2), 256, 257, 258, 259):
        check(lib().sdk_probe_copy_ex(_ptr(src), _ptr(dst), nbytes, mode, _stream()), "probe_copy")
        best = float("inf")
        for _ in range(reps):
            e0, e1 = torch.cuda.Event(enable_timing=True), torch.cuda.Event(enable_timing=True)
            e0.record()
            check(lib().sdk_probe_copy_ex(_ptr(src), _ptr(dst), nbytes, mode, _stream()), "probe_copy")
            e1.record()
            e1.synchronize()
            best = min(best, e0.elapsed_time(e1))
        gbs = 2 * nbytes / (best * 1e-3) / 1e9
        if gbs > best_gbs:
            best_gbs, best_mode = gbs, mode
    out["hbm_copy_gbs"] = round(best_gbs, 1)
    out["hbm_copy_mode"] = {"loads_in_flight": 8 if best_mode & 1 else 4, "nontemporal": bool(best_mode & 2),
                            "form": "flat one pass" if best_mode & 256 else "grid-stride",
                            "workgroups_per_cu": None if best_mode & 256 else ((best_mode >> 2) & 63) or 16}
    del src, dst
    return out



ATTN_FORMS = {"auto": _lib.ATTN_AUTO, "nw4": _lib.ATTN_NW4, "nw8": _lib.ATTN_NW8, "nw8_stag": _lib.ATTN_NW8_STAG,
              "qb2": _lib.ATTN_QB2, "wide": _lib.ATTN_WIDE}
_ATTN_FORM_NAMES = {v: k for k, v in ATTN_FORMS.items()}
ATTN_WIDE_ROWS = _lib.ATTN_WIDE_ROWS
ATTN_WIDE_KT = _lib.ATTN_WIDE_KT


def attention(q, k, v, *, batch, heads, nq, nk, head_dim, scale, out=None, causal=False, form=None, form_out=None):
    for t, n in ((q, "q"), (k, "k"), (v, "v")):
        _need_cuda(t, "attention " + n)
    if out is None:
        out = torch.empty(batch * nq, heads * head_dim, dtype=torch.float16, device=q.device)
    _claim(out)
    a = AttentionArgs()
    a.q, a.k, a.v, a.o = q.data_ptr(), k.data_ptr(), v.data_ptr(), out.data_ptr()
    a.q_ld, a.k_ld, a.v_ld, a.o_ld = q.stride(0), k.stride(0), v.stride(0), out.stride(0)
    a.batch, a.heads, a.nq, a.nk, a.head_dim, a.scale = batch, heads, nq, nk, head_dim, scale
    a.causal = 1 if causal else 0
    if PROFILER.active:
        PROFILER.begin("attention", (batch, heads, nq, nk, head_dim))
    if form is None and form_out is None:
        check(lib().sdk_attention(C.byref(a), _stream()), "attention")
    else:
        info = _lib.AttentionFormInfo()
        check(lib().sdk_attention_form(C.byref(a), ATTN_FORMS[form or "auto"], C.byref(info), _stream()), "attention")
        if form_out is not None:
            form_out.update(form=_ATTN_FORM_NAMES[info.form], dqk=info.dqk, dv=info.dv, waves=info.waves,
                            qblocks=info.qblocks, stagger=info.stagger, seed_col=info.seed_col,
                            causal=info.causal, grid=info.grid)
    if PROFILER.active:
        PROFILER.end()
    return out


def linear_attention(q, k, v, *, batch, heads, n, dim_head, out=None):
    for t, nm in ((q, "q"), (k, "k"), (v, "v")):
        _need_cuda(t, "linear_attention " + nm)
    if out is None:
        out = torch.empty(batch * n, heads * dim_head, dtype=torch.float16, device=q.device)
    _claim(out)
    a = _lib.LinearAttentionArgs()
    a.q, a.k, a.v, a.o = q.data_ptr(), k.data_ptr(), v.data_ptr(), out.data_ptr()
    a.q_ld, a.k_ld, a.v_ld, a.o_ld = q.stride(0), k.stride(0), v.stride(0), out.stride(0)
    a.batch, a.heads, a.n, a.dim_head = batch, heads, n, dim_head
    nbytes = lib().sdk_linear_attention_workspace_bytes(C.byref(a))
    if nbytes < 0:
        check(-1, "linear_attention")
    ws = torch.empty(nbytes, dtype=torch.uint8, device=q.device)
    a.workspace, a.workspace_bytes = ws.data_ptr(), nbytes
    if PROFILER.active:
        PROFILER.begin("linear_attention", None)
    check(lib().sdk_linear_attention(C.byref(a), _stream()), "linear_attention")
    if PROFILER.active:
        PROFILER.end()
    return out


def cross_attention_block_supported(channels, head_dim, nk, n_img):
    return bool(lib().sdk_cross_attention_block_supported(channels, head_dim, nk, n_img))


XATTN_PACKED_W = True


def xattn_packed_weight(pc: PackedConv):
    pk = getattr(pc, "_xattn_pk", None)
    if pk is None:
        Cc = pc.N
        pk = torch.empty(Cc * Cc, dtype=torch.float16, device=pc.weight.device)
        check(lib().sdk_xattn_pack_weight(pc.weight.data_ptr(), pc.k_total, pk.data_ptr(), Cc, _stream()),
              "xattn_pack_weight")
        pc._xattn_pk = pk
    return pk


def cross_attention_block(t, kv, pc_q: PackedConv, pc_o: PackedConv, *, batch, n_img, nk, heads, head_dim, scale,
                          residual=None, out=None, norm_in=None, norm_out=None, out_ln=None):
    Cc = heads * head_dim
    for x, n in ((t, "t"), (kv, "kv")):
        _need_cuda(x, "cross_attention_block " + n)
    if pc_q.k_total != Cc or pc_o.k_total != Cc or pc_q.N != Cc or pc_o.N != Cc:
        raise ValueError("sd_amd.cross_attention_block: to_q / to_out must be channels x channels")
    if out is None:
        out = torch.empty(batch * n_img, Cc, dtype=torch.float16, device=t.device)
    _claim(out)
    _claim(out_ln)
    a = XAttnArgs()
    a.t, a.kv, a.wq, a.wo = t.data_ptr(), kv.data_ptr(), pc_q.weight.data_ptr(), pc_o.weight.data_ptr()
    packed = XATTN_PACKED_W and (not torch.cuda.is_current_stream_capturing() or
                                 (hasattr(pc_q, "_xattn_pk") and hasattr(pc_o, "_xattn_pk")))
    if packed:
        a.wq, a.wo = xattn_packed_weight(pc_q).data_ptr(), xattn_packed_weight(pc_o).data_ptr()
    a.bias = pc_o.bias.data_ptr() if pc_o.bias is not None else None
    a.res = residual.data_ptr() if residual is not None else None
    a.out = out.data_ptr()
    a.t_ld, a.kv_ld, a.w_ld = t.stride(0), kv.stride(0), 0 if packed else Cc
    a.res_ld = residual.stride(0) if residual is not None else 0
    a.out_ld = out.stride(0)
    a.batch, a.n_img, a.nk, a.channels, a.head_dim, a.scale = batch, n_img, nk, Cc, head_dim, scale
    if PROFILER.active:
        PROFILER.begin("cross_attention_block", None)
        PROFILER._cur = PROFILER._cur[:2] + (4.0 * batch * n_img * Cc * Cc + 4.0 * batch * n_img * nk * Cc,) + \
            PROFILER._cur[3:]
    if norm_in is None and norm_out is None:
        check(lib().sdk_cross_attention_block(C.byref(a), _stream()), "cross_attention_block")
    else:
        ln = XAttnLnArgs()
        if norm_in is not None:
            ln.in_gamma, ln.in_beta, ln.in_eps = norm_in[0].data_ptr(), norm_in[1].data_ptr(), norm_in[2]
        if norm_out is not None:
            if out_ln is None:
                out_ln = torch.empty_like(out)
            ln.out_gamma, ln.out_beta, ln.out_eps = norm_out[0].data_ptr(), norm_out[1].data_ptr(), norm_out[2]
            ln.out_ln, ln.out_ln_ld = out_ln.data_ptr(), out_ln.stride(0)
        check(lib().sdk_cross_attention_block_ln(C.byref(a), C.byref(ln), _stream()), "cross_attention_block")
    if PROFILER.active:
        PROFILER.end()
    return (out, out_ln) if norm_out is not None else out


def ff_supported(channels, features):
    return bool(lib().sdk_ff_supported(channels, features))


class PackedFF:

    def __init__(self, w1, b1, w2, b2, device):
        F2, Cc = w1.shape
        self.channels, self.features = Cc, F2 // 2
        if not ff_supported(Cc, self.features):
            raise ValueError(f"sd_amd.PackedFF: unsupported shape channels={Cc} features={self.features}")
        w1h = w1.detach().to(device=device, dtype=torch.float16).contiguous()
        w2h = w2.detach().to(device=device, dtype=torch.float16).contiguous()
        b1f = b1.detach().to(device=device, dtype=torch.float32).contiguous() if b1 is not None else None
        self.b2 = b2.detach().to(device=device, dtype=torch.float32).contiguous() if b2 is not None else None
        nbytes = lib().sdk_ff_packed_bytes(Cc, self.features)
        self.packed = torch.empty(nbytes, dtype=torch.uint8, device=device)
        check(lib().sdk_ff_pack(_ptr(w1h), _ptr(b1f), _ptr(w2h), _ptr(self.packed), Cc, self.features, _stream()),
              "ff_pack")


def feed_forward(pf: PackedFF, t, residual=None, out=None):
    _need_cuda(t, "feed_forward t")
    M, Cc = t.shape
    if Cc != pf.channels or t.stride(-1) != 1:
        raise ValueError("sd_amd.feed_forward: t must be [M, channels] with unit column stride")
    if out is None:
        out = torch.empty(M, Cc, dtype=torch.float16, device=t.device)
    _claim(out)
    a = FfArgs()
    a.t, a.out, a.packed = t.data_ptr(), out.data_ptr(), pf.packed.data_ptr()
    a.b2 = pf.b2.data_ptr() if pf.b2 is not None else None
    if residual is not None:
        _need_cuda(residual, "feed_forward residual")
        a.res, a.res_ld = residual.data_ptr(), residual.stride(0)
    a.t_ld, a.out_ld = t.stride(0), out.stride(0)
    a.rows, a.channels, a.features = M, Cc, pf.features
    if PROFILER.active:
        PROFILER.begin("feed_forward", None, shape=(M, Cc, pf.features))
        PROFILER._cur = PROFILER._cur[:2] + (2.0 * M * Cc * 3 * pf.features,) + PROFILER._cur[3:]
    check(lib().sdk_feed_forward(C.byref(a), _stream()), "feed_forward")
    if PROFILER.active:
        PROFILER.end()
    return out


def token_linear_supported(in_features, out_features):
    return bool(lib().sdk_token_linear_supported(in_features, out_features))


class PackedTokenLinear:

    def __init__(self, w, b, device):
        w = w.detach().reshape(w.shape[0], -1)
        if not token_linear_supported(w.shape[1], w.shape[0]):
            raise ValueError(f"sd_amd.PackedTokenLinear: unsupported shape {tuple(w.shape)}")
        self.features = w.shape[0]
        self.w = w.to(device=device, dtype=torch.float16).contiguous()
        self.b = b.detach().to(device=device, dtype=torch.float32).contiguous() if b is not None else None


def token_linear(pk: PackedTokenLinear, x, residual=None, out=None, norm=None):
    _need_cuda(x, "token_linear x")
    M, K = x.shape
    if K != pk.features or x.stride(-1) != 1:
        raise ValueError("sd_amd.token_linear: x must be [M, 320] with unit column stride")
    if out is None:
        out = torch.empty(M, pk.features, dtype=torch.float16, device=x.device)
    _claim(out)
    a = TokenLinearArgs()
    a.x, a.w, a.out = x.data_ptr(), pk.w.data_ptr(), out.data_ptr()
    a.bias = pk.b.data_ptr() if pk.b is not None else None
    if residual is not None:
        _need_cuda(residual, "token_linear residual")
        if residual.shape != (M, pk.features) or residual.stride(-1) != 1:
            raise ValueError("sd_amd.token_linear: residual must be [M, 320] with unit column stride")
        a.res, a.res_ld = residual.data_ptr(), residual.stride(0)
    a.x_ld, a.out_ld = x.stride(0), out.stride(0)
    a.rows, a.in_features, a.out_features = M, K, pk.features
    if PROFILER.active:
        PROFILER.begin("token_linear", None, shape=(M, pk.features, K))
        PROFILER._cur = PROFILER._cur[:2] + (2.0 * M * K * pk.features,) + PROFILER._cur[3:]
    if norm is None:
        check(lib().sdk_token_linear(C.byref(a), _stream()), "token_linear")
    else:
        g, bt, eps = norm
        _need_cuda(g, "token_linear_ln gamma", torch.float32)
        _need_cuda(bt, "token_linear_ln beta", torch.float32)
        if g.numel() != pk.features or bt.numel() != pk.features:
            raise ValueError("sd_amd.token_linear: norm gamma / beta must have 320 elements")
        out_ln = torch.empty(M, pk.features, dtype=torch.float16, device=x.device)
        check(lib().sdk_token_linear_ln(C.byref(a), g.data_ptr(), bt.data_ptr(), float(eps), out_ln.data_ptr(),
                                        out_ln.stride(0), _stream()), "token_linear_ln")
    if PROFILER.active:
        PROFILER.end()
    return out if norm is None else (out, out_ln)



def token_embedding(ids: torch.Tensor, tok: torch.Tensor, pos: torch.Tensor):
    _need_cuda(ids, "token_embedding", torch.int64)
    _need_cuda(tok, "token_embedding table", torch.float32)
    _need_cuda(pos, "token_embedding positions", torch.float32)
    B, T = ids.shape
    if T > pos.shape[0]:
        raise ValueError(f"sd_amd.token_embedding: {T} tokens > {pos.shape[0]} positions")
    out = torch.empty(B, T, tok.shape[1], dtype=torch.float16, device=ids.device)
    check(lib().sdk_token_embedding(_ptr(ids.contiguous()), _ptr(tok), _ptr(pos), _ptr(out), B, T, tok.shape[1],
                                    _stream()), "token_embedding")
    return out


def extract_patches(z: torch.Tensor, kh: int, kw: int, sy: int, sx: int):
    _need_cuda(z, "extract_patches", torch.float32)
    z = z.contiguous()
    B, Cc, H, W = z.shape
    Ly, Lx = (H - kh) // sy + 1, (W - kw) // sx + 1
    out = torch.empty(Ly * Lx, B, Cc, kh, kw, dtype=torch.float32, device=z.device)
    check(lib().sdk_extract_patches(_ptr(z), _ptr(out), B, Cc, H, W, kh, kw, sy, sx, _stream()), "extract_patches")
    return out


def fold_patches(patches: torch.Tensor, pix_w: torch.Tensor, l_w, H: int, W: int, sy: int, sx: int, Ly: int,
                 Lx: int):
    _need_cuda(patches, "fold_patches", torch.float32)
    _need_cuda(pix_w, "fold_patches weights", torch.float32)
    patches = patches.contiguous()
    L, B, Cc, ph, pw = patches.shape
    assert L == Ly * Lx
    out = torch.empty(B, Cc, H, W, dtype=torch.float32, device=patches.device)
    check(lib().sdk_fold_patches(_ptr(patches), _ptr(pix_w.contiguous()), _ptr(l_w), _ptr(out), B, Cc, H, W, ph, pw,
                                 sy, sx, Ly, Lx, _stream()), "fold_patches")
    return out


def timestep_embedding(t: torch.Tensor, freqs: torch.Tensor, dim: int):
    _need_cuda(t, "timestep_embedding", torch.int64)
    out = torch.empty(t.shape[0], dim, dtype=torch.float16, device=t.device)
    check(lib().sdk_timestep_embedding(_ptr(t), _ptr(freqs), _ptr(out), t.shape[0], dim, _stream()),
          "timestep_embedding")
    return out


def nchw_to_nhwc(x: torch.Tensor, c_pad: int, scale: float = 1.0):
    _need_cuda(x, "nchw_to_nhwc", torch.float32)
    x = x.contiguous()
    B, Cc, H, W = x.shape
    y = torch.empty(B, H, W, c_pad, dtype=torch.float16, device=x.device)
    check(lib().sdk_nchw_to_nhwc(_ptr(x), _ptr(y), B, Cc, H * W, c_pad, C.c_float(scale), _stream()),
          "nchw_to_nhwc")
    return y


def _drop_scale(what, keep, drop_p, ref, noise):
    p = float(drop_p)
    if not 0.0 <= p <= 1.0:
        raise ValueError(f"sd_amd.{what}: drop_p must be in [0, 1], got {drop_p}")
    if keep is None:
        if p > 0.0:
            raise ValueError(f"sd_amd.{what}: drop_p > 0 needs keep (one byte per element)")
        return None, 0.0
    if not torch.is_tensor(keep) or not keep.is_cuda or keep.device != ref.device or \
            keep.dtype not in (torch.uint8, torch.bool):
        raise ValueError(f"sd_amd.{what}: keep must be a CUDA uint8 / bool tensor on {ref.device}")
    if keep.shape != ref.shape:
        raise ValueError(f"sd_amd.{what}: keep {tuple(keep.shape)} vs {tuple(ref.shape)}")
    if noise is None:
        raise ValueError(f"sd_amd.{what}: keep needs noise")
    keep = keep.contiguous()
    if keep.dtype == torch.bool:
        keep = keep.view(torch.uint8)
    return keep, (0.0 if p == 1.0 else float(np.float32(1.0 / (1.0 - p))))


def _same_f32(what, ref, **tensors):
    out = {}
    for k, v in tensors.items():
        if v is None:
            out[k] = None
            continue
        if not torch.is_tensor(v) or not v.is_cuda or v.dtype != torch.float32 or v.device != ref.device:
            raise ValueError(f"sd_amd.{what}: {k} must be a CUDA fp32 tensor on {ref.device}")
        if v.shape != ref.shape:
            raise ValueError(f"sd_amd.{what}: {k} {tuple(v.shape)} vs {tuple(ref.shape)}")
        out[k] = v.contiguous()
    return out


def _mask_mode(what, mask, shape):
    if len(shape) != 4:
        raise ValueError(f"sd_amd.{what}: the mask blend needs NCHW tensors, got {tuple(shape)}")
    B, Cc, H, W = shape
    modes = {(B, 1, H, W): 0, (1, 1, H, W): 1, (B, Cc, H, W): 2}
    if tuple(mask.shape) not in modes:
        raise ValueError(f"sd_amd.{what}: mask {tuple(mask.shape)} does not broadcast over {tuple(shape)}")
    return modes[tuple(mask.shape)]


def _ddim_ex(what, ref, x, e, sc, pred_x0_in, noise, e_uncond, guidance, v_param, x_prev, pred_x0, temperature,
             keep, drop_p, blend_x0, blend_noise, blend_mask, blend_sqrt_acp, blend_sqrt_1m_acp, x_next):
    t = _same_f32(what, ref, noise=noise, e_uncond=e_uncond)
    noise, e_uncond = t["noise"], t["e_uncond"]
    keep, scale = _drop_scale(what, keep, drop_p, ref, noise)
    ex = _lib.DdimExArgs()
    a = ex.step
    a.x = x.data_ptr() if x is not None else None
    a.e, a.x_prev, a.pred_x0 = e.data_ptr(), x_prev.data_ptr(), pred_x0.data_ptr()
    a.e_uncond = e_uncond.data_ptr() if e_uncond is not None else None
    a.noise = noise.data_ptr() if noise is not None else None
    a.n = ref.numel()
    if not pred_x0_in:
        a.sqrt_one_minus_at = float(sc["sqrt_one_minus_at"])
        a.sqrt_at = float(sc["sqrt_at"])
    a.dir_coef = float(sc["dir_coef"])
    a.sqrt_a_prev = float(sc["sqrt_a_prev"])
    a.sigma = float(sc["sigma"])
    a.temperature = float(temperature)
    a.guidance = float(guidance)
    if v_param is not None:
        a.v_param = 1
        a.v_sqrt_a, a.v_sqrt_1ma = float(v_param[0]), float(v_param[1])
    ex.pred_x0_in = int(pred_x0_in)
    if keep is not None:
        ex.keep, ex.drop_scale = keep.data_ptr(), scale
    if blend_mask is None:
        if blend_x0 is not None or blend_noise is not None or x_next is not None:
            raise ValueError(f"sd_amd.{what}: blend_x0 / blend_noise / x_next need blend_mask")
        check(lib().sdk_ddim_step_ex(C.byref(ex), _stream()), what)
        return None
    if blend_x0 is None or blend_noise is None or blend_sqrt_acp is None or blend_sqrt_1m_acp is None:
        raise ValueError(f"sd_amd.{what}: the blend needs blend_x0, blend_noise, blend_sqrt_acp and blend_sqrt_1m_acp")
    t = _same_f32(what, ref, blend_x0=blend_x0, blend_noise=blend_noise)
    if not torch.is_tensor(blend_mask) or not blend_mask.is_cuda or blend_mask.dtype != torch.float32 or \
            blend_mask.device != ref.device:
        raise ValueError(f"sd_amd.{what}: blend_mask must be a CUDA fp32 tensor on {ref.device}")
    m = ex.blend
    m.mask_mode = _mask_mode(what, blend_mask, ref.shape)
    blend_mask = blend_mask.contiguous()
    if x_next is None:
        x_next = torch.empty_like(ref)
    elif x_next.shape != ref.shape or not x_next.is_contiguous() or x_next.dtype != torch.float32 or \
            x_next.device != ref.device:
        raise ValueError(f"sd_amd.{what}: x_next must be a contiguous CUDA fp32 tensor of x's shape")
    m.x0, m.noise, m.mask, m.out = t["blend_x0"].data_ptr(), t["blend_noise"].data_ptr(), blend_mask.data_ptr(), \
        x_next.data_ptr()
    m.n, m.per_sample, m.hw = ref.numel(), ref.numel() // ref.shape[0], ref.shape[2] * ref.shape[3]
    m.sqrt_acp, m.sqrt_1m_acp = float(blend_sqrt_acp), float(blend_sqrt_1m_acp)
    check(lib().sdk_ddim_step_ex(C.byref(ex), _stream()), what)
    return x_next


def ddim_step(x, e, sc: dict, noise=None, e_uncond=None, guidance=1.0, v_param=None, x_prev=None, pred_x0=None,
              temperature=1.0, *, keep=None, drop_p=0.0, blend_x0=None, blend_noise=None, blend_mask=None,
              blend_sqrt_acp=None, blend_sqrt_1m_acp=None, x_next=None):
    _need_cuda(x, "ddim_step", torch.float32)
    _need_cuda(e, "ddim_step", torch.float32)
    if e.shape != x.shape:
        raise ValueError(f"sd_amd.ddim_step: x {tuple(x.shape)} vs e {tuple(e.shape)}")
    x, e = x.contiguous(), e.contiguous()
    xp = x_prev if x_prev is not None else torch.empty_like(x)
    p0 = pred_x0 if pred_x0 is not None else torch.empty_like(x)
    xn = _ddim_ex("ddim_step", x, x, e, sc, False, noise, e_uncond, guidance, v_param, xp, p0, temperature, keep,
                  drop_p, blend_x0, blend_noise, blend_mask, blend_sqrt_acp, blend_sqrt_1m_acp, x_next)
    return (xp, p0) if xn is None else (xp, p0, xn)


def ddim_xprev(pred_x0, e, sc: dict, x=None, noise=None, e_uncond=None, guidance=1.0, v_param=None, x_prev=None,
               temperature=1.0, *, keep=None, drop_p=0.0, blend_x0=None, blend_noise=None, blend_mask=None,
               blend_sqrt_acp=None, blend_sqrt_1m_acp=None, x_next=None):
    _need_cuda(pred_x0, "ddim_xprev", torch.float32)
    _need_cuda(e, "ddim_xprev", torch.float32)
    if e.shape != pred_x0.shape:
        raise ValueError(f"sd_amd.ddim_xprev: pred_x0 {tuple(pred_x0.shape)} vs e {tuple(e.shape)}")
    pred_x0, e = pred_x0.contiguous(), e.contiguous()
    xp = x_prev if x_prev is not None else torch.empty_like(pred_x0)
    if v_param is not None:
        if x is None:
            raise ValueError("sd_amd.ddim_xprev: v_param needs x")
        _need_cuda(x, "ddim_xprev", torch.float32)
        x = x.contiguous()
    else:
        x = None
    xn = _ddim_ex("ddim_xprev", pred_x0, x, e, sc, True, noise, e_uncond, guidance, v_param, xp, pred_x0, temperature,
                  keep, drop_p, blend_x0, blend_noise, blend_mask, blend_sqrt_acp, blend_sqrt_1m_acp, x_next)
    return xp if xn is None else (xp, xn)


MULTISTEP_FORMS = {"plms": _lib.MULTISTEP_PLMS, "plms_warmup": _lib.MULTISTEP_PLMS_WARMUP, "dpm": _lib.MULTISTEP_DPM}


def multistep_step(x, e, sc: dict, form="plms", history=(), e_next=None, coefs=None, e_uncond=None, guidance=1.0,
                   v_param=None, x_prev=None, pred_x0=None, hist_out=None, *, blend_x0=None, blend_noise=None,
                   blend_mask=None, blend_sqrt_acp=None, blend_sqrt_1m_acp=None, x_next=None):
    what = "multistep_step"
    _need_cuda(x, what, torch.float32)
    _need_cuda(e, what, torch.float32)
    if e.shape != x.shape:
        raise ValueError(f"sd_amd.{what}: x {tuple(x.shape)} vs e {tuple(e.shape)}")
    if form not in MULTISTEP_FORMS:
        raise ValueError(f"sd_amd.{what}: form must be one of {sorted(MULTISTEP_FORMS)}, got {form!r}")
    history = list(history)
    most = {"plms": 3, "plms_warmup": 0, "dpm": 1}[form]
    if len(history) > most:
        raise ValueError(f"sd_amd.{what}: form '{form}' takes at most {most} history tensors, got {len(history)}")
    if (form == "plms_warmup") != (e_next is not None):
        raise ValueError(f"sd_amd.{what}: e_next goes with form 'plms_warmup' (and only with it)")
    if (form == "dpm") != (coefs is not None):
        raise ValueError(f"sd_amd.{what}: coefs = (c_x, c_0, c_1) goes with form 'dpm' (and only with it)")
    x, e = x.contiguous(), e.contiguous()
    t = _same_f32(what, x, e_uncond=e_uncond, e_next=e_next, **{f"history[{k}]": h for k, h in enumerate(history)})
    for k, h in enumerate(history):
        if h is None:
            raise ValueError(f"sd_amd.{what}: history[{k}] is None")
    outs = {"x_prev": x_prev, "pred_x0": pred_x0, "hist_out": hist_out, "x_next": x_next}
    for k, v in outs.items():
        if v is not None and (not torch.is_tensor(v) or v.shape != x.shape or not v.is_contiguous() or
                              v.dtype != torch.float32 or v.device != x.device):
            raise ValueError(f"sd_amd.{what}: {k} must be a contiguous CUDA fp32 tensor of x's shape")
    xp = x_prev if x_prev is not None else torch.empty_like(x)
    p0 = pred_x0 if pred_x0 is not None else torch.empty_like(x)
    m = _lib.MultistepArgs()
    a = m.step
    a.x, a.e, a.x_prev, a.pred_x0 = x.data_ptr(), e.data_ptr(), xp.data_ptr(), p0.data_ptr()
    a.e_uncond = t["e_uncond"].data_ptr() if t["e_uncond"] is not None else None
    a.n = x.numel()
    a.sqrt_one_minus_at, a.sqrt_at = float(sc["sqrt_one_minus_at"]), float(sc["sqrt_at"])
    if form != "dpm":
        if float(sc.get("sigma", 0.0)) != 0.0:
            raise ValueError(f"sd_amd.{what}: PLMS is deterministic: the scalars must be those of eta = 0")
        a.dir_coef, a.sqrt_a_prev = float(sc["dir_coef"]), float(sc["sqrt_a_prev"])
    else:
        m.c_x, m.c_0, m.c_1 = (float(c) for c in coefs)
    a.temperature, a.guidance = 1.0, float(guidance)
    if v_param is not None:
        a.v_param = 1
        a.v_sqrt_a, a.v_sqrt_1ma = float(v_param[0]), float(v_param[1])
    m.form, m.nhist = MULTISTEP_FORMS[form], len(history)
    for k in range(len(history)):
        m.hist[k] = t[f"history[{k}]"].data_ptr()
    if e_next is not None:
        m.e_next = t["e_next"].data_ptr()
    if hist_out is not None:
        m.hist_out = hist_out.data_ptr()
    if blend_mask is None:
        if blend_x0 is not None or blend_noise is not None or x_next is not None:
            raise ValueError(f"sd_amd.{what}: blend_x0 / blend_noise / x_next need blend_mask")
        check(lib().sdk_multistep_step(C.byref(m), _stream()), what)
        return xp, p0
    if blend_x0 is None or blend_noise is None or blend_sqrt_acp is None or blend_sqrt_1m_acp is None:
        raise ValueError(f"sd_amd.{what}: the blend needs blend_x0, blend_noise, blend_sqrt_acp and blend_sqrt_1m_acp")
    tb = _same_f32(what, x, blend_x0=blend_x0, blend_noise=blend_noise)
    if not torch.is_tensor(blend_mask) or not blend_mask.is_cuda or blend_mask.dtype != torch.float32 or \
            blend_mask.device != x.device:
        raise ValueError(f"sd_amd.{what}: blend_mask must be a CUDA fp32 tensor on {x.device}")
    b = m.blend
    b.mask_mode = _mask_mode(what, blend_mask, x.shape)
    blend_mask = blend_mask.contiguous()
    xn = x_next if x_next is not None else torch.empty_like(x)
    b.x0, b.noise, b.mask, b.out = tb["blend_x0"].data_ptr(), tb["blend_noise"].data_ptr(), blend_mask.data_ptr(), \
        xn.data_ptr()
    b.n, b.per_sample, b.hw = x.numel(), x.numel() // x.shape[0], x.shape[2] * x.shape[3]
    b.sqrt_acp, b.sqrt_1m_acp = float(blend_sqrt_acp), float(blend_sqrt_1m_acp)
    check(lib().sdk_multistep_step(C.byref(m), _stream()), what)
    return xp, p0, xn


def cfg_combine(e_uncond, e_cond, guidance, out=None):
    _need_cuda(e_cond, "cfg_combine", torch.float32)
    t = _same_f32("cfg_combine", e_cond, e_uncond=e_uncond)
    if t["e_uncond"] is None:
        raise ValueError("sd_amd.cfg_combine: e_uncond must be a CUDA fp32 tensor")
    e_cond = e_cond.contiguous()
    y = out if out is not None else torch.empty_like(e_cond)
    if y.shape != e_cond.shape or not y.is_contiguous() or y.dtype != torch.float32 or y.device != e_cond.device:
        raise ValueError("sd_amd.cfg_combine: out must be a contiguous CUDA fp32 tensor of e_cond's shape")
    check(lib().sdk_cfg_combine(t["e_uncond"].data_ptr(), e_cond.data_ptr(), y.data_ptr(), e_cond.numel(),
                                C.c_float(float(guidance)), _stream()), "cfg_combine")
    return y



def concat_nchw_to_nhwc(srcs, c_pad: int):
    srcs = list(srcs)
    if not 1 <= len(srcs) <= 4:
        raise ValueError(f"sd_amd.concat_nchw_to_nhwc: 1..4 sources, got {len(srcs)}")
    for s in srcs:
        _need_cuda(s, "concat_nchw_to_nhwc", torch.float32)
        if s.dim() != 4 or s.shape[0] != srcs[0].shape[0] or s.shape[2:] != srcs[0].shape[2:]:
            raise ValueError("sd_amd.concat_nchw_to_nhwc: sources must be NCHW with the same batch and spatial "
                             f"size, got {[tuple(t.shape) for t in srcs]}")
    srcs = [s.contiguous() for s in srcs]
    B, _, H, W = srcs[0].shape
    csum = sum(s.shape[1] for s in srcs)
    if c_pad < csum:
        raise ValueError(f"sd_amd.concat_nchw_to_nhwc: c_pad {c_pad} below the channel sum {csum}")
    y = torch.empty(B, H, W, c_pad, dtype=torch.float16, device=srcs[0].device)
    a = _lib.ConcatArgs()
    for i, s in enumerate(srcs):
        a.src[i], a.channels[i] = s.data_ptr(), s.shape[1]
    a.nsrc, a.y, a.batch, a.hw, a.c_pad = len(srcs), y.data_ptr(), B, H * W, c_pad
    check(lib().sdk_concat_nchw_to_nhwc(C.byref(a), _stream()), "concat_nchw_to_nhwc")
# ... 312 lines not shown
```

stable-diffusion-from-scratch_amd/packing.py:

```python
from __future__ import annotations

import os

import torch
from torch import nn

from . import ops


class PackedOwner:

    _packed_key = None
    prepare_generation = 0

    def _load_from_state_dict(self, *args, **kwargs):
        self.invalidate_packed()
        return super()._load_from_state_dict(*args, **kwargs)

    def invalidate_packed(self):
        self._packed_key = None
        self.prepare_generation += 1
        self._packs_dropped()

    def _packs_dropped(self):
        """Per-class hook: drop what was derived from the packs just invalidated."""

    @torch.no_grad()
    def repack(self, *key, **pack_args):
        self.invalidate_packed()
        self._pack(*key, **pack_args)
        self._packed_key = key

    def ensure_packed(self, *key, **pack_args):
        if self._packed_key != key:
            self.repack(*key, **pack_args)


def f32(param, dev):
    return param.detach().to(dev, torch.float32).contiguous()


def prep_norm(norm, dev):
    norm._g = f32(norm.weight, dev)
    norm._b = f32(norm.bias, dev)


def gn_affine(gn, x):
    return ops.group_norm_affine(x, gn._g, gn._b, gn.eps, gn.num_groups)


def gn_norm(gn, x, silu=True, pad=0):
    return ops.group_norm(x, gn._g, gn._b, gn.eps, gn.num_groups, silu=silu, pad=pad)


def pack_res_tail(conv2, skip, cin, cout, dev):
    if isinstance(skip, nn.Conv2d) and skip.kernel_size[0] == 1:
        return "fused", ops.PackedConv([(conv2.weight, cout), (skip.weight, cin)],
                                       conv2.bias.detach() + skip.bias.detach(), device=dev), None
    pc2 = ops.PackedConv([(conv2.weight, cout)], conv2.bias, device=dev)
    if isinstance(skip, nn.Conv2d):
        return "conv3", pc2, ops.PackedConv([(skip.weight, cin)], skip.bias, device=dev)
    return "identity", pc2, None


def run_res_tail(tail, ha, x, pad):
    mode, pc2, pc_skip = tail
    if mode == "identity":
        return ops.conv2d(pc2, ha, pad=pad, residual=x, gn_stats=True)
    if mode == "fused":
        return ops.conv2d(pc2, ha, pad=pad, seg2=(x, None, False), gn_stats=True)
    return ops.conv2d(pc2, ha, pad=pad, residual=ops.conv2d(pc_skip, x), gn_stats=True)


UPSAMPLE_FOLD = os.environ.get("SD_AMD_UPSAMPLE_FOLD", "0") == "1"
UPSAMPLE_MATERIALISE = os.environ.get("SD_AMD_UPSAMPLE_MATERIALISE", "0") == "1"


def upsample_phase_ok(x, padding=1):
    return not (UPSAMPLE_FOLD or UPSAMPLE_MATERIALISE) and not isinstance(x, tuple) and x.shape[-1] % 64 == 0 \
        and padding == 1


def pack_upsample_conv(conv, channels, dev, padding=1):
    pc = ops.PackedConv([(conv.weight, channels)], conv.bias, device=dev)
    ppc = None
    if channels % 64 == 0 and padding == 1 and not (UPSAMPLE_FOLD or UPSAMPLE_MATERIALISE):
        ppc = ops.PhaseConv(conv.weight, channels, conv.bias, device=dev)
    return pc, ppc


def run_upsample_conv(pc, ppc, x, padding=1, materialise_max_bytes=None):
    if ppc is not None and upsample_phase_ok(x, padding):
        return ops.conv2d(ppc, ops.zero_border(x, 1), phase=True, gn_stats=True)
    fold = UPSAMPLE_FOLD or isinstance(x, tuple) or x.shape[-1] % 8 != 0
    if not fold and materialise_max_bytes is not None:
        n, h, w, c = x.shape
        fold = n * (2 * h + 2) * (2 * w + 2) * c * 2 > materialise_max_bytes
    if fold:
        return ops.conv2d(pc, x, upsample=True, pad=padding, gn_stats=True)
    return ops.conv2d(pc, ops.upsample_nearest2x_padded(x, padding), pad=0, gn_stats=True)
```

Baseline: 18.02 images/sec.

## Fuse transformer proj_in, LayerNorm and QKV projection into one chained kernel

Adds a fused HIP kernel for 320-channel spatial transformers. In one pass per row panel it applies the group-norm scale/shift, runs the proj_in GEMM, applies norm1 LayerNorm and then the fused QKV GEMM, writing both the token tensor and qkv. The goal is to avoid separate launches and the HBM round trips of the intermediate normalized and projected activations. It relies on a permuted proj_in weight layout and a CU-fill heuristic for when to use the chain, and it only applies to the 320-channel blocks.

```diff
diff --git a/include/sdk_amd.h b/include/sdk_amd.h
--- a/include/sdk_amd.h
+++ b/include/sdk_amd.h
@@ -209,6 +209,17 @@
                         void* out_ln, int32_t out_ln_ld, sdk_stream_t stream);
 
 typedef struct {
+  const void* x; const float* gn_scale; const float* gn_shift; const void* w; const float* bias;
+  const float* gamma; const float* beta; void* tok; void* qkv;
+  int32_t x_ld, tok_ld, qkv_ld, rows, hw;
+  int32_t in_features, features, qkv_features;
+  float eps;
+} sdk_proj_norm_qkv_args;
+
+int sdk_proj_norm_qkv_supported(int32_t in_features, int32_t features, int32_t qkv_features);
+int sdk_proj_norm_qkv(const sdk_proj_norm_qkv_args* a, sdk_stream_t stream);
+
+typedef struct {
   const float* x; const float* e; const float* e_uncond; const float* noise;
   float* x_prev; float* pred_x0;
   int64_t n;
diff --git a/stable-diffusion-from-scratch_amd/_lib.py b/stable-diffusion-from-scratch_amd/_lib.py
--- a/stable-diffusion-from-scratch_amd/_lib.py
+++ b/stable-diffusion-from-scratch_amd/_lib.py
@@ -79,6 +79,12 @@
 class TokenLinearArgs(C.Structure):
     _fields_ = [("x", vp), ("w", vp), ("bias", vp), ("res", vp), ("out", vp), ("x_ld", i32), ("res_ld", i32),
                 ("out_ld", i32), ("rows", i32), ("in_features", i32), ("out_features", i32)]
+
+
+class ProjNormQkvArgs(C.Structure):
+    _fields_ = [("x", vp), ("gn_scale", vp), ("gn_shift", vp), ("w", vp), ("bias", vp), ("gamma", vp), ("beta", vp),
+                ("tok", vp), ("qkv", vp), ("x_ld", i32), ("tok_ld", i32), ("qkv_ld", i32), ("rows", i32), ("hw", i32),
+                ("in_features", i32), ("features", i32), ("qkv_features", i32), ("eps", f32)]
 
 
 class DdimArgs(C.Structure):
@@ -139,7 +145,7 @@
 GN_APPLY = ("none", "in_stats", "flat", "row", "stride")
 
 EXPORTS = ["sdk_conv2d_plan", "sdk_conv2d", "sdk_group_norm_workspace", "sdk_group_norm_affine", "sdk_group_norm_apply", "sdk_group_norm_apply_padded", "sdk_group_norm_apply_ex", "sdk_group_norm", "sdk_group_norm_finalize", "sdk_group_norm_plan", "sdk_layer_norm",
-           "sdk_attention", "sdk_attention_form", "sdk_linear_attention", "sdk_linear_attention_workspace_bytes", "sdk_linear_attention_chunks", "sdk_cross_attention_block_supported", "sdk_xattn_pack_weight", "sdk_cross_attention_block", "sdk_cross_attention_block_ln", "sdk_segment_softmax", "sdk_ff_supported", "sdk_ff_packed_bytes", "sdk_ff_pack", "sdk_feed_forward", "sdk_token_linear_supported", "sdk_token_linear", "sdk_token_linear_ln", "sdk_ddim_step", "sdk_ddim_xprev", "sdk_ddim_step_ex", "sdk_multistep_step", "sdk_cfg_combine", "sdk_posterior_step", "sdk_posterior_step_ex", "sdk_masked_q_sample", "sdk_concat_nchw_to_nhwc", "sdk_patch_pack", "sdk_ddpm_step", "sdk_timestep_embedding", "sdk_nchw_to_nhwc",
+           "sdk_attention", "sdk_attention_form", "sdk_linear_attention", "sdk_linear_attention_workspace_bytes", "sdk_linear_attention_chunks", "sdk_cross_attention_block_supported", "sdk_xattn_pack_weight", "sdk_cross_attention_block", "sdk_cross_attention_block_ln", "sdk_segment_softmax", "sdk_ff_supported", "sdk_ff_packed_bytes", "sdk_ff_pack", "sdk_feed_forward", "sdk_token_linear_supported", "sdk_token_linear", "sdk_token_linear_ln", "sdk_proj_norm_qkv_supported", "sdk_proj_norm_qkv", "sdk_ddim_step", "sdk_ddim_xprev", "sdk_ddim_step_ex", "sdk_multistep_step", "sdk_cfg_combine", "sdk_posterior_step", "sdk_posterior_step_ex", "sdk_masked_q_sample", "sdk_concat_nchw_to_nhwc", "sdk_patch_pack", "sdk_ddpm_step", "sdk_timestep_embedding", "sdk_nchw_to_nhwc",
            "sdk_diag_gaussian_sample", "sdk_stochastic_encode", "sdk_token_embedding", "sdk_extract_patches",
            "sdk_fold_patches", "sdk_vq_code_norms", "sdk_vq_nearest_splits", "sdk_vq_nearest", "sdk_vq_lookup", "sdk_vq_remap",
            "sdk_upsample_bilinear2x", "sdk_upsample_nearest2x_padded", "sdk_zero_border", "sdk_gelu",
@@ -200,6 +206,8 @@
     L.sdk_token_linear_supported.argtypes = [i32, i32]
     L.sdk_token_linear.argtypes = [C.POINTER(TokenLinearArgs), vp]
     L.sdk_token_linear_ln.argtypes = [C.POINTER(TokenLinearArgs), vp, vp, f32, vp, i32, vp]
+    L.sdk_proj_norm_qkv_supported.argtypes = [i32, i32, i32]
+    L.sdk_proj_norm_qkv.argtypes = [C.POINTER(ProjNormQkvArgs), vp]
     L.sdk_ddim_step.argtypes = [C.POINTER(DdimArgs), vp]
     L.sdk_ddim_xprev.argtypes = [C.POINTER(DdimArgs), vp]
     L.sdk_posterior_step.argtypes = [C.POINTER(PosteriorArgs), vp]
diff --git a/stable-diffusion-from-scratch_amd/build.py b/stable-diffusion-from-scratch_amd/build.py
--- a/stable-diffusion-from-scratch_amd/build.py
+++ b/stable-diffusion-from-scratch_amd/build.py
@@ -9,7 +9,7 @@
 CSRC = os.path.join(HERE, "csrc")
 BUILD = os.path.join(HERE, "build")
 LIB = os.path.join(HERE, "libsdk_amd.so")
-SOURCES = ["norm.hip", "attention.hip", "attention_wide.hip", "linattn.hip", "sampler.hip", "xattn.hip", "ff.hip", "token.hip", "vq.hip", "cond.hip", "probe.hip"]
+SOURCES = ["norm.hip", "attention.hip", "attention_wide.hip", "linattn.hip", "sampler.hip", "xattn.hip", "ff.hip", "token.hip", "proj_qkv.hip", "vq.hip", "cond.hip", "probe.hip"]
 CONV_TILE_PARTS = 5
 
 
@@ -25,7 +25,7 @@
 
 def _deps(src: str, csrc: str):
     headers = [os.path.join(csrc, "common.h"), os.path.join(HERE, "..", "include", "sdk_amd.h")]
-    if src.startswith("conv"):
+    if src.startswith("conv") or src == "proj_qkv.hip":
         headers += sorted(os.path.join(csrc, f) for f in os.listdir(csrc) if f.startswith("conv") and f.endswith(".h"))
     return [os.path.join(csrc, src)] + headers
 HIPCC = os.environ.get("HIPCC", "/opt/rocm/bin/hipcc")
@@ -33,7 +33,7 @@
 EXTRA = {"attention.hip": ["-mno-amdgpu-ieee", "-fno-honor-nans"],
          "attention_wide.hip": ["-mno-amdgpu-ieee", "-fno-honor-nans"]}
 REMARK = "-Rpass-analysis=kernel-resource-usage"
-NO_SCRATCH = re.compile(r"token_linear320_kernel|attn_wide_kernel|conv_rowpanel_kernel")
+NO_SCRATCH = re.compile(r"token_linear320_kernel|attn_wide_kernel|conv_rowpanel_kernel|proj_norm_qkv_kernel")
 WARN_SCRATCH = re.compile(r"conv_glds_kernel|conv_ph_kernel|ff_geglu_kernel|xattn_block_kernel|attn_fwd_kernel|vq_nearest_")
 _RES = re.compile(r"remark: (?:Function Name: (\S+)|\s+(VGPRs|AGPRs|ScratchSize \[bytes/lane\]|Occupancy \[waves/SIMD\]): (\d+))")
 
diff --git a/stable-diffusion-from-scratch_amd/csrc/common.h b/stable-diffusion-from-scratch_amd/csrc/common.h
--- a/stable-diffusion-from-scratch_amd/csrc/common.h
+++ b/stable-diffusion-from-scratch_amd/csrc/common.h
@@ -34,6 +34,11 @@
 }
 
 __device__ __forceinline__ float silu_f(float x) { return x / (1.0f + __expf(-x)); }
+__device__ __forceinline__ float gn_act(float x, float sc, float sh, int silu) {
+  float t = x * sc + sh;
+  if (silu) t = t * __builtin_amdgcn_rcpf(1.0f + __expf(-t));
+  return t;
+}
 __device__ __forceinline__ float erf_fast(float x) {
   const float a = fabsf(x);
   const float t = __builtin_amdgcn_rcpf(fmaf(0.3275911f, a, 1.0f));
@@ -102,10 +107,23 @@
   rstd = rsqrtf(var + eps);
 }
 
-template <int CPL>
-__device__ __forceinline__ void ln_quad_stats(const h8 (&v)[CPL], float eps, float& mean, float& rstd) {
+struct LnQuadLanes {
+  static __device__ __forceinline__ float pivot(float x) { return dpp_f<0x00>(x); }
+  static __device__ __forceinline__ float x1(float x) { return dpp_f<0xB1>(x); }
+  static __device__ __forceinline__ float x2(float x) { return dpp_f<0x4E>(x); }
+};
+struct LnFragLanes {
+  static __device__ __forceinline__ float from(float x, int l) {
+    return __builtin_bit_cast(float, __builtin_amdgcn_ds_bpermute(4 * l, __builtin_bit_cast(int, x)));
+  }
+  static __device__ __forceinline__ float pivot(float x) { return from(x, threadIdx.x & 15); }
+  static __device__ __forceinline__ float x1(float x) { return from(x, (threadIdx.x & 63) ^ 16); }
+  static __device__ __forceinline__ float x2(float x) { return from(x, (threadIdx.x & 63) ^ 32); }
+};
+template <int CPL, class X>
+__device__ __forceinline__ void ln_quad_stats_on(const h8 (&v)[CPL], float eps, float& mean, float& rstd) {
 #pragma clang fp contract(off)
-  const float x0 = dpp_f<0x00>((float)v[0][0]);
+  const float x0 = X::pivot((float)v[0][0]);
   float s1 = 0.f, s2 = 0.f;
 #pragma unroll
   for (int i = 0; i < CPL; ++i)
@@ -115,15 +133,19 @@
       s1 += d;
       s2 = __builtin_fmaf(d, d, s2);
     }
-  s1 += dpp_f<0xB1>(s1);
-  s2 += dpp_f<0xB1>(s2);
-  s1 += dpp_f<0x4E>(s1);
-  s2 += dpp_f<0x4E>(s2);
+  s1 += X::x1(s1);
+  s2 += X::x1(s2);
+  s1 += X::x2(s1);
+  s2 += X::x2(s2);
   const float inv_n = 1.f / (32 * CPL);
   const float dm = s1 * inv_n;
   const float var = fmaxf(__builtin_fmaf(-dm, dm, s2 * inv_n), 0.f);
   mean = x0 + dm;
   rstd = rsqrtf(var + eps);
+}
+template <int CPL>
+__device__ __forceinline__ void ln_quad_stats(const h8 (&v)[CPL], float eps, float& mean, float& rstd) {
+  ln_quad_stats_on<CPL, LnQuadLanes>(v, eps, mean, rstd);
 }
 
 __device__ __forceinline__ h8 ln_quad_apply(const h8& v, float mean, float rstd, const float* gb, int C, int k) {
diff --git a/stable-diffusion-from-scratch_amd/csrc/norm.hip b/stable-diffusion-from-scratch_amd/csrc/norm.hip
--- a/stable-diffusion-from-scratch_amd/csrc/norm.hip
+++ b/stable-diffusion-from-scratch_amd/csrc/norm.hip
@@ -36,12 +36,6 @@
   const f4 a = q[0], b = q[1];
 #pragma unroll
   for (int j = 0; j < 4; ++j) { o[j] = a[j]; o[4 + j] = b[j]; }
-}
-
-__device__ __forceinline__ float gn_act(float x, float sc, float sh, int silu) {
-  float t = x * sc + sh;
-  if (silu) t = t * __builtin_amdgcn_rcpf(1.0f + __expf(-t));
-  return t;
 }
 
 __device__ __forceinline__ h8 gn_act8(h8 v, const float sc[8], const float sh[8], int silu) {
diff --git a/stable-diffusion-from-scratch_amd/csrc/proj_qkv.hip b/stable-diffusion-from-scratch_amd/csrc/proj_qkv.hip
--- /dev/null
+++ b/stable-diffusion-from-scratch_amd/csrc/proj_qkv.hip
@@ -0,0 +1,332 @@
+#include "conv_cfg.h"
+#include "conv_device.h"
+
+namespace sdk {
+namespace {
+
+using RP = CfgRowPanel;
+constexpr int RP_NW = 8, RP_NT = RP_NW * 64;
+constexpr int RP_TG = RP::TBM / RP_NW / 16;
+constexpr int RP_NB = RP::TBN / 16;
+constexpr int RP_KS = RP::MAXK / 32;
+constexpr int RP_KT = (RP::MAXK + BK - 1) / BK;
+constexpr int RP_SLOT_H = RP::TBN * BK;
+constexpr int RP_PIECES = RP::TBN / 8;
+constexpr int RP_PPW = (RP_PIECES + RP_NW - 1) / RP_NW;
+constexpr int RP_NS = 5;
+constexpr int RP_PFD = 4;
+constexpr int RP_RS = RP::TBN + 8;
+constexpr int RP_SCR = 16 * RP_RS * 2;
+constexpr int RP_CPR = RP::TBN / 8;
+constexpr int RP_CPT = 16 * RP_CPR / 64;
+constexpr unsigned RP_OOB = 0x80000000u;
+constexpr int RP_EST = RP_TG * RP_CPT;
+constexpr int PQ_C = 320, PQ_NQKV = 960, PQ_N = PQ_C + PQ_NQKV;
+constexpr int PQ_NCH = PQ_N / RP::TBN, PQ_NCH_IN = PQ_C / RP::TBN;
+constexpr int RP_OFF_DUMMY = RP_NS * RP_SLOT_H * 2;
+constexpr int RP_OFF_SCR = RP_OFF_DUMMY + 1024;
+constexpr int PQ_OFF_BIAS = RP_OFF_SCR + RP_NW * RP_SCR;
+constexpr int PQ_OFF_GB = PQ_OFF_BIAS + PQ_N * 4;
+constexpr int PQ_LDS = PQ_OFF_GB + 2 * PQ_C * 4;
+static_assert(RP::TBM == RP_NW * 16 * RP_TG && RP::TBN % 16 == 0 && RP::MAXK % 32 == 0, "whole MFMA blocks");
+static_assert(16 * RP_CPR % 64 == 0, "whole read-back instructions per 16-row block");
+static_assert((RP_NS - 2) * RP_PPW + RP_EST <= 63, "vmcnt immediate");
+static_assert(RP_NS - 1 <= RP_KT, "at most one epilogue between a slot's pieces and its wait");
+static_assert(RP::MAXK == PQ_C && PQ_C % RP::TBN == 0 && PQ_NQKV % RP::TBN == 0 && PQ_C == RP_KT * BK, "whole chunks and slots");
+static_assert(RP_NB % 2 == 0, "two accumulator blocks per operand fragment");
+static_assert(PQ_LDS <= 160 * 1024, "LDS");
+
+__device__ __forceinline__ __amdgpu_buffer_rsrc_t rp_rsrc(const void* base, long long bytes) {
+  const int n = (int)(bytes < 0x7fffffffLL ? bytes : 0x7fffffffLL);
+  return __builtin_amdgcn_make_buffer_rsrc(const_cast<void*>(base), 0, n, 0x00020000);
+}
+
+template <int G, int g = 0>
+__device__ __forceinline__ void rp_pin_groups() {
+  if constexpr (g < G) {
+    if constexpr (g + RP_PFD < G) __builtin_amdgcn_sched_group_barrier(0x100, 1, 0);
+    __builtin_amdgcn_sched_group_barrier(0x008, RP_TG, 0);
+    if constexpr (g < RP_PPW) __builtin_amdgcn_sched_group_barrier(0x020, 1, 0);
+    rp_pin_groups<G, g + 1>();
+  }
+}
+
+template <bool PERM>
+__device__ __forceinline__ void pq_rows16(const f4* a, half_t* wbuf, const float* bias_c, __amdgpu_buffer_rsrc_t ro,
+                                          const unsigned (&voff)[RP_CPT], h4* keep = nullptr) {
+  const int lane = threadIdx.x & 63, px = lane & 15, cg = lane >> 4;
+#pragma unroll
+  for (int j = 0; j < RP_NB; ++j) {
+    const f4 bb = *reinterpret_cast<const f4*>(bias_c + 16 * j + 4 * cg);
+    h4 o;
+#pragma unroll
+    for (int q = 0; q < 4; ++q) o[q] = (half_t)(a[j][q] + bb[q]);
+    if constexpr (PERM) keep[j] = o;
+    const int col = PERM ? 32 * (j / 2) + 8 * cg + 4 * (j % 2) : 16 * j + 4 * cg;
+    *reinterpret_cast<h4*>(wbuf + px * RP_RS + col) = o;
+  }
+#pragma unroll
+  for (int i = 0; i < RP_CPT; ++i) {
+    const int idx = lane + 64 * i, row = idx / RP_CPR, ch = idx - row * RP_CPR;
+    const h8 v = *reinterpret_cast<const h8*>(wbuf + row * RP_RS + ch * 8);
+    __builtin_amdgcn_raw_buffer_store_b128(__builtin_bit_cast(__attribute__((ext_vector_type(4))) unsigned, v), ro,
+                                           voff[i], 0, 0);
+  }
+}
+
+struct ChainParams {
+  const half_t* x; const float* gn_scale; const float* gn_shift; const half_t* w; const float* bias;
+  const float* gamma; const float* beta; half_t* tok; half_t* qkv;
+  int x_ld, tok_ld, qkv_ld, M, hw, nimg;
+  float eps;
+};
+
+template <bool GN>
+__global__ void __launch_bounds__(RP_NT, 2) proj_norm_qkv_kernel(ChainParams p) {
+  extern __shared__ __attribute__((aligned(16))) half_t lds[];
+  char* const ldsb = reinterpret_cast<char*>(lds);
+  half_t* const dummy = reinterpret_cast<half_t*>(ldsb + RP_OFF_DUMMY);
+  float* const bias_s = reinterpret_cast<float*>(ldsb + PQ_OFF_BIAS);
+  float* const gb = reinterpret_cast<float*>(ldsb + PQ_OFF_GB);
+  const int tid = threadIdx.x, lane = tid & 63;
+  const int wave = __builtin_amdgcn_readfirstlane(tid >> 6);
+  __builtin_assume(wave >= 0 && wave < RP_NW);
+  const int r16 = lane & 15, kq = lane >> 4;
+  const int m0 = (int)blockIdx.x * RP::TBM;
+  const int rows = min(RP::TBM, p.M - m0);
+  constexpr int ldw = PQ_C;
+
+  for (int n = tid; n < PQ_N; n += RP_NT) bias_s[n] = p.bias[n];
+  for (int n = tid; n < PQ_C; n += RP_NT) {
+    gb[n] = p.gamma[n];
+    gb[PQ_C + n] = p.beta[n];
+  }
+
+  const __amdgpu_buffer_rsrc_t rw = rp_rsrc(p.w, (long long)PQ_N * ldw * 2);
+  const int prow0 = wave * 8 + (lane >> 3);
+  const unsigned vb0 = (unsigned)(prow0 * ldw) * 2u + (unsigned)((lane & 7) ^ ((prow0 >> 1) & 7)) * 16u;
+  int ic = 0, ikt = 0, ipos = 0;
+  auto issue_piece = [&](int j) __attribute__((always_inline)) {
+    const unsigned off = (unsigned)((ic * RP::TBN + j * 8 * RP_NW) * ldw + ikt * BK) * 2u;
+    const int piece = j * RP_NW + wave;
+    half_t* dst = piece < RP_PIECES ? lds + ipos * RP_SLOT_H + piece * 8 * BK : dummy;
+    __builtin_amdgcn_raw_ptr_buffer_load_lds(rw, (__attribute__((address_space(3))) void*)dst, 16,
+                                             piece < RP_PIECES && ic < PQ_NCH ? vb0 + off : RP_OOB, 0, 0, 0);
+  };
+  auto issue_next = [&]() __attribute__((always_inline)) {
+    if (++ikt == RP_KT) {
+      ikt = 0;
+      ++ic;
+    }
+    ipos = ipos + 1 == RP_NS ? 0 : ipos + 1;
+  };
+#pragma unroll
+  for (int s = 0; s < RP_NS - 1; ++s) {
+#pragma unroll
+    for (int j = 0; j < RP_PPW; ++j) issue_piece(j);
+    issue_next();
+  }
+
+  const __amdgpu_buffer_rsrc_t ra = rp_rsrc(p.x + (size_t)m0 * p.x_ld, ((long long)(rows - 1) * p.x_ld + PQ_C) * 2);
+  h8 xf[RP_KS][RP_TG];
+#pragma unroll
+  for (int ks = 0; ks < RP_KS; ++ks)
+#pragma unroll
+    for (int tg = 0; tg < RP_TG; ++tg) {
+      const unsigned row = (unsigned)(32 * wave + 16 * tg + r16);
+      xf[ks][tg] = __builtin_bit_cast(
+          h8, __builtin_amdgcn_raw_buffer_load_b128(ra, (row * (unsigned)p.x_ld + 8u * kq) * 2u + 64u * ks, 0, 0));
+    }
+  if constexpr (GN) {
+    const __amdgpu_buffer_rsrc_t rsc = rp_rsrc(p.gn_scale, (long long)p.nimg * PQ_C * 4);
+    const __amdgpu_buffer_rsrc_t rsh = rp_rsrc(p.gn_shift, (long long)p.nimg * PQ_C * 4);
+    unsigned goff[RP_TG];
+#pragma unroll
+    for (int tg = 0; tg < RP_TG; ++tg)
+      goff[tg] = (unsigned)(((m0 + 32 * wave + 16 * tg + r16) / p.hw) * PQ_C + 8 * kq) * 4u;
+#pragma unroll
+    for (int ks = 0; ks < RP_KS; ++ks)
+#pragma unroll
+      for (int tg = 0; tg < RP_TG; ++tg) {
+        const unsigned o = goff[tg] + 128u * ks;
+        const f4 sc0 = __builtin_bit_cast(f4, __builtin_amdgcn_raw_buffer_load_b128(rsc, o, 0, 0));
+        const f4 sc1 = __builtin_bit_cast(f4, __builtin_amdgcn_raw_buffer_load_b128(rsc, o + 16u, 0, 0));
+        const f4 sh0 = __builtin_bit_cast(f4, __builtin_amdgcn_raw_buffer_load_b128(rsh, o, 0, 0));
+        const f4 sh1 = __builtin_bit_cast(f4, __builtin_amdgcn_raw_buffer_load_b128(rsh, o + 16u, 0, 0));
+        h8 v = xf[ks][tg];
+#pragma unroll
+        for (int j = 0; j < 4; ++j) {
+          v[j] = (half_t)gn_act((float)v[j], sc0[j], sh0[j], 0);
+          v[4 + j] = (half_t)gn_act((float)v[4 + j], sc1[j], sh1[j], 0);
+        }
+        xf[ks][tg] = v;
+      }
+  }
+#pragma unroll
+  for (int ks = 0; ks < RP_KS; ++ks)
+#pragma unroll
+    for (int tg = 0; tg < RP_TG; ++tg) asm volatile("" : "+v"(xf[ks][tg]));
+  asm volatile("s_waitcnt lgkmcnt(0)" ::: "memory");
+
+  half_t* const wscr = reinterpret_cast<half_t*>(ldsb + RP_OFF_SCR + wave * RP_SCR);
+  const __amdgpu_buffer_rsrc_t rt =
+      rp_rsrc(p.tok + (size_t)m0 * p.tok_ld, ((long long)(rows - 1) * p.tok_ld + PQ_C) * 2);
+  const __amdgpu_buffer_rsrc_t rq =
+      rp_rsrc(p.qkv + (size_t)m0 * p.qkv_ld, ((long long)(rows - 1) * p.qkv_ld + PQ_NQKV) * 2);
+
+  int rpos = 0;
+  auto chunk = [&](f4 (&acc)[RP_TG][RP_NB], const h8 (&b)[RP_KS][RP_TG], bool late) __attribute__((always_inline)) {
+#pragma unroll
+    for (int tg = 0; tg < RP_TG; ++tg)
+#pragma unroll
+      for (int nb = 0; nb < RP_NB; ++nb) acc[tg][nb] = f4{};
+#pragma unroll
+    for (int kt = 0; kt < RP_KT; ++kt) {
+      __builtin_amdgcn_sched_barrier(0);
+      if (late && kt < RP_KT - 1)
+        asm volatile("s_waitcnt vmcnt(%0)" ::"n"((RP_NS - 2) * RP_PPW + RP_EST) : "memory");
+      else
+        asm volatile("s_waitcnt vmcnt(%0)" ::"n"((RP_NS - 2) * RP_PPW) : "memory");
+      __builtin_amdgcn_sched_barrier(0);
+      __builtin_amdgcn_s_barrier();
+      __builtin_amdgcn_sched_barrier(0);
+      const half_t* st = lds + rpos * RP_SLOT_H;
+      constexpr int G = (BK / 32) * RP_NB;
+      auto rd = [&](int gq) __attribute__((always_inline)) {
+        return *reinterpret_cast<const h8*>(st + swz(16 * (gq % RP_NB) + r16, 4 * (gq / RP_NB) + kq));
+      };
+      h8 wq[RP_PFD + 1];
+#pragma unroll
+      for (int gq = 0; gq < RP_PFD; ++gq) wq[gq] = rd(gq);
+#pragma unroll
+      for (int gq = 0; gq < G; ++gq) {
+        if (gq + RP_PFD < G) wq[(gq + RP_PFD) % (RP_PFD + 1)] = rd(gq + RP_PFD);
+        const int nb = gq % RP_NB;
+#pragma unroll
+        for (int tg = 0; tg < RP_TG; ++tg)
+          acc[tg][nb] = __builtin_amdgcn_mfma_f32_16x16x32_f16(wq[gq % (RP_PFD + 1)], b[2 * kt + gq / RP_NB][tg],
+                                                               acc[tg][nb], 0, 0, 0);
+        if (gq < RP_PPW) issue_piece(gq);
+      }
+      issue_next();
+      __builtin_amdgcn_sched_group_barrier(0x100, RP_PFD, 0);
+      rp_pin_groups<G>();
+      rpos = rpos + 1 == RP_NS ? 0 : rpos + 1;
+    }
+  };
+  auto offsets = [&](unsigned (&vo)[RP_CPT], int tg, int ld, int n0) __attribute__((always_inline)) {
+    int l = lane;
+    asm volatile("" : "+v"(l));
+#pragma unroll
+    for (int i = 0; i < RP_CPT; ++i) {
+      const int idx = l + 64 * i, row = idx / RP_CPR;
+      vo[i] = (unsigned)((32 * wave + 16 * tg + row) * ld + n0 + (idx - row * RP_CPR) * 8) * 2u;
+    }
+  };
+
+  h8 tf[RP_KS][RP_TG];
+#pragma unroll
+  for (int c = 0; c < PQ_NCH_IN; ++c) {
+    f4 acc[RP_TG][RP_NB];
+    chunk(acc, xf, c > 0);
+#pragma unroll
+    for (int tg = 0; tg < RP_TG; ++tg) {
+      unsigned vo[RP_CPT];
+      offsets(vo, tg, p.tok_ld, c * RP::TBN);
+      h4 keep[RP_NB];
+      pq_rows16<true>(acc[tg], wscr, bias_s + c * RP::TBN, rt, vo, keep);
+#pragma unroll
+      for (int i = 0; i < RP_NB / 2; ++i) {
+        h8& f = tf[c * (RP_NB / 2) + i][tg];
+        f = __builtin_shufflevector(keep[2 * i], keep[2 * i + 1], 0, 1, 2, 3, 4, 5, 6, 7);
+        asm volatile("" : "+v"(f));
+      }
+    }
+  }
+
+  __builtin_amdgcn_sched_barrier(0);
+  int kql = kq;
+  asm volatile("" : "+v"(kql));
+#pragma unroll
+  for (int tg = 0; tg < RP_TG; ++tg) {
+    h8 v[RP_KS];
+#pragma unroll
+    for (int ks = 0; ks < RP_KS; ++ks) v[ks] = tf[ks][tg];
+    float mean, rstd;
+    ln_quad_stats_on<RP_KS, LnFragLanes>(v, p.eps, mean, rstd);
+#pragma unroll
+    for (int ks = 0; ks < RP_KS; ++ks) xf[ks][tg] = ln_quad_apply(v[ks], mean, rstd, gb, PQ_C, kql + 4 * ks);
+  }
+  __builtin_amdgcn_sched_barrier(0);
+
+#pragma unroll 1
+  for (int c = PQ_NCH_IN; c < PQ_NCH; ++c) {
+    f4 acc[RP_TG][RP_NB];
+    chunk(acc, xf, true);
+#pragma unroll
+    for (int tg = 0; tg < RP_TG; ++tg) {
+      unsigned vo[RP_CPT];
+      offsets(vo, tg, p.qkv_ld, (c - PQ_NCH_IN) * RP::TBN);
+      pq_rows16<false>(acc[tg], wscr, bias_s + c * RP::TBN, rq, vo);
+    }
+  }
+  asm volatile("s_waitcnt vmcnt(0)" ::: "memory");
+}
+
+template <bool GN>
+int proj_norm_qkv_launch(const ChainParams& p, hipStream_t s) {
+  static std::atomic<unsigned long long> attr_set{0};
+  if (int e = ensure_dyn_lds((const void*)proj_norm_qkv_kernel<GN>, PQ_LDS, attr_set, "proj_norm_qkv")) return e;
+  hipLaunchKernelGGL((proj_norm_qkv_kernel<GN>), dim3((p.M + RP::TBM - 1) / RP::TBM), dim3(RP_NT), PQ_LDS, s, p);
+  return check_launch("proj_norm_qkv");
+}
+
+bool pq_overlap(const void* a, long long ab, const void* b, long long bb) {
+  const char *a0 = (const char*)a, *b0 = (const char*)b;
+  return a0 < b0 + bb && b0 < a0 + ab;
+}
+
+}
+}
+
+using namespace sdk;
+
+extern "C" int sdk_proj_norm_qkv_supported(int32_t in_features, int32_t features, int32_t qkv_features) {
+  return in_features == PQ_C && features == PQ_C && qkv_features == PQ_NQKV ? 1 : 0;
+}
+
+extern "C" int sdk_proj_norm_qkv(const sdk_proj_norm_qkv_args* a, sdk_stream_t stream) {
+  if (!a || !a->x || !a->w || !a->bias || !a->gamma || !a->beta || !a->tok || !a->qkv)
+    return fail(SDK_EINVAL, "proj_norm_qkv: null pointer");
+  if (!sdk_proj_norm_qkv_supported(a->in_features, a->features, a->qkv_features))
+    return fail(SDK_EINVAL, "proj_norm_qkv: in_features / features / qkv_features must be 320 / 320 / 960");
+  if (a->rows <= 0) return fail(SDK_EINVAL, "proj_norm_qkv: empty");
+  if (a->x_ld % 8 || a->tok_ld % 8 || a->qkv_ld % 8 || a->x_ld < PQ_C || a->tok_ld < PQ_C || a->qkv_ld < PQ_NQKV)
+    return fail(SDK_EINVAL, "proj_norm_qkv: row strides must be multiples of 8 and at least the row widths");
+  if (((uintptr_t)a->x | (uintptr_t)a->w | (uintptr_t)a->bias | (uintptr_t)a->gamma | (uintptr_t)a->beta |
+       (uintptr_t)a->tok | (uintptr_t)a->qkv | (uintptr_t)a->gn_scale | (uintptr_t)a->gn_shift) & 15)
+    return fail(SDK_EINVAL, "proj_norm_qkv: pointers must be 16-B aligned");
+  const bool gn = a->gn_scale || a->gn_shift;
+  if (gn && (!a->gn_scale || !a->gn_shift || a->hw <= 0 || a->rows % a->hw))
+    return fail(SDK_EINVAL, "proj_norm_qkv: a GroupNorm affine needs scale, shift and hw (rows a multiple of hw)");
+  if (a->x_ld > (1 << 20) || a->tok_ld > (1 << 20) || a->qkv_ld > (1 << 20))
+    return fail(SDK_EINVAL, "proj_norm_qkv: row stride too large");
+  const long long xb = ((long long)(a->rows - 1) * a->x_ld + PQ_C) * 2;
+  const long long tb = ((long long)(a->rows - 1) * a->tok_ld + PQ_C) * 2;
+  const long long qb = ((long long)(a->rows - 1) * a->qkv_ld + PQ_NQKV) * 2;
+  const long long gbytes = gn ? (long long)(a->rows / a->hw) * PQ_C * 4 : 0;
+  const struct { const void* p; long long n; } in[] = {{a->x, xb}, {a->w, (long long)PQ_N * PQ_C * 2}, {a->bias, PQ_N * 4},
+                                                        {a->gamma, PQ_C * 4}, {a->beta, PQ_C * 4},
+                                                        {a->gn_scale, gbytes}, {a->gn_shift, gbytes}};
+  for (const auto& i : in)
+    if (i.p && (pq_overlap(i.p, i.n, a->tok, tb) || pq_overlap(i.p, i.n, a->qkv, qb)))
+      return fail(SDK_EINVAL, "proj_norm_qkv: an output overlaps an input");
+  if (pq_overlap(a->tok, tb, a->qkv, qb)) return fail(SDK_EINVAL, "proj_norm_qkv: tok and qkv overlap");
+  ChainParams p;
+  p.x = (const half_t*)a->x; p.gn_scale = a->gn_scale; p.gn_shift = a->gn_shift;
+  p.w = (const half_t*)a->w; p.bias = a->bias; p.gamma = a->gamma; p.beta = a->beta;
+  p.tok = (half_t*)a->tok; p.qkv = (half_t*)a->qkv;
+  p.x_ld = a->x_ld; p.tok_ld = a->tok_ld; p.qkv_ld = a->qkv_ld; p.M = a->rows;
+  p.hw = gn ? a->hw : 1; p.nimg = gn ? a->rows / a->hw : 0; p.eps = a->eps;
+  return gn ? proj_norm_qkv_launch<true>(p, (hipStream_t)stream) : proj_norm_qkv_launch<false>(p, (hipStream_t)stream);
+}
diff --git a/stable-diffusion-from-scratch_amd/openai_model/attention.py b/stable-diffusion-from-scratch_amd/openai_model/attention.py
--- a/stable-diffusion-from-scratch_amd/openai_model/attention.py
+++ b/stable-diffusion-from-scratch_amd/openai_model/attention.py
@@ -7,7 +7,7 @@
 from torch import nn
 
 from .. import ops
-from ..packing import f32, gn_norm, prep_norm
+from ..packing import f32, gn_norm, gn_scale_shift, prep_norm
 from .utils import conv_nd, normalization, zero_module
 
 
@@ -39,6 +39,9 @@
 
 FUSED_FF = os.environ.get("SD_AMD_FUSED_FF") != "0"
 TOKEN_LINEAR = os.environ.get("SD_AMD_TOKEN_LINEAR", "1") != "0"
+_CHAIN_ENV = os.environ.get("SD_AMD_PROJ_QKV_CHAIN", "1")
+PROJ_QKV_CHAIN = _CHAIN_ENV != "0"
+PROJ_QKV_CHAIN_GN = _CHAIN_ENV != "xn"
 
 
 class ReassocContext:
@@ -130,11 +133,12 @@
             return ops.PerImageWeights(w1, H * L), ops.PerImageWeights(w2, Co, self._bo32)
         return ReassocContext(kv, H, L, B, build)
 
-    def _run(self, t, residual, B, N, kv=None, Lc=None):
+    def _run(self, t, residual, B, N, kv=None, Lc=None, qkv=None):
         inner = self.heads * self.dim_head
         if kv is None:
             if self.self_attn:
-                qkv = ops.linear(self._pc_qkv, t)
+                if qkv is None:
+                    qkv = ops.linear(self._pc_qkv, t)
                 q, k, v, nk = qkv[:, :inner], qkv[:, inner:2 * inner], qkv[:, 2 * inner:], N
             else:
                 q = ops.linear(self._pc_q, t)
@@ -220,10 +224,10 @@
         for n in (self.norm1, self.norm2, self.norm3):
             prep_norm(n, dev)
 
-    def _run(self, tok, B, N, kv=None, Lc=None, t=None):
-        if t is None:
+    def _run(self, tok, B, N, kv=None, Lc=None, t=None, qkv=None):
+        if t is None and qkv is None:
             t = ops.layer_norm(tok, self.norm1._g, self.norm1._b, self.norm1.eps)
-        tok = self.attn1._run(t, tok, B, N)
+        tok = self.attn1._run(t, tok, B, N, qkv=qkv)
         a2 = self.attn2
         if (kv is not None and FUSED_XATTN_NORMS and tok.stride(-1) == 1
                 and _use_fused_xattn(a2.heads * a2.dim_head, a2.dim_head, Lc, N, B)):
@@ -269,12 +273,30 @@
         self._pc_out = ops.PackedConv([(self.proj_out.weight, self.inner_dim)], self.proj_out.bias, device=dev)
         for blk in self.transformer_blocks:
             blk._prepare(dev)
+        self._ppq = None
+        if len(self.transformer_blocks) and self._ptl_in is not None:
+            a1 = self.transformer_blocks[0].attn1
+            if ops.proj_norm_qkv_supported(self.in_channels, self.inner_dim, 3 * a1.heads * a1.dim_head):
+                wqkv = torch.cat([a1.to_q.weight, a1.to_k.weight, a1.to_v.weight], 0)
+                self._ppq = ops.PackedProjQkv(self.proj_in.weight, self.proj_in.bias, wqkv, dev)
 
     def context_kv(self, ctx2d, L=None):
         return [blk.attn2.context_kv(ctx2d, L) for blk in self.transformer_blocks]
 
     def _run(self, x, kvs=None, Lc=None):
         B, H, W, Cc = x.shape
+        if (PROJ_QKV_CHAIN and TOKEN_LINEAR and self._ppq is not None and x.is_contiguous()
+                and ops.proj_qkv_chain_fills(B * H * W, ops.cu_count(x.device))):
+            n1 = self.transformer_blocks[0].norm1
+            if PROJ_QKV_CHAIN_GN:
+                tok, qkv = ops.proj_norm_qkv(self._ppq, x.view(B * H * W, Cc), (n1._g, n1._b, n1.eps),
+                                             gn=gn_scale_shift(self.norm, x), hw=H * W)
+            else:
+                xn = gn_norm(self.norm, x, silu=False)
+                tok, qkv = ops.proj_norm_qkv(self._ppq, xn.view(B * H * W, Cc), (n1._g, n1._b, n1.eps))
+            for i, blk in enumerate(self.transformer_blocks):
+                tok = blk._run(tok, B, H * W, None if kvs is None else kvs[i], Lc, qkv=qkv if i == 0 else None)
+            return ops.conv2d(self._pc_out, tok.view(B, H, W, self.inner_dim), residual=x, gn_stats=True)
         xn = gn_norm(self.norm, x, silu=False)
         t1 = None
         if TOKEN_LINEAR and self._ptl_in is not None and xn.is_contiguous():
diff --git a/stable-diffusion-from-scratch_amd/ops.py b/stable-diffusion-from-scratch_amd/ops.py
--- a/stable-diffusion-from-scratch_amd/ops.py
+++ b/stable-diffusion-from-scratch_amd/ops.py
@@ -7,7 +7,7 @@
 import torch
 
 from . import _lib
-from ._lib import (ACT_NONE, ACT_QUICK_GELU, ACT_GELU, AttentionArgs, XAttnArgs, XAttnLnArgs, FfArgs, TokenLinearArgs, ConvArgs, ConvPlanInfo, GroupNormArgs,
+from ._lib import (ACT_NONE, ACT_QUICK_GELU, ACT_GELU, AttentionArgs, XAttnArgs, XAttnLnArgs, FfArgs, TokenLinearArgs, ProjNormQkvArgs, ConvArgs, ConvPlanInfo, GroupNormArgs,
                    OUT_GEGLU_F16, OUT_NCHW_F32, OUT_NHWC_F16, OUT_ROWS_F32, check, lib)
 
 BK = 64
@@ -1102,6 +1102,105 @@
     return out if norm is None else (out, out_ln)
 
 
+PROJ_QKV_C, PROJ_QKV_N = 320, 960
+PROJ_QKV_PANEL = 256
+
+
+def proj_qkv_perm():
+    p = torch.arange(PROJ_QKV_C)
+    c, r = p // 160, p % 160
+    nb, cg, q = r // 16, (r % 16) // 4, r % 4
+    g = 10 * c + nb
+    return 32 * (g // 2) + 8 * cg + 4 * (g % 2) + q
+
+
+def proj_qkv_pack(w_in, b_in, w_qkv, b_qkv=None):
+    w_in = w_in.detach().float().reshape(w_in.shape[0], -1)
+    w_qkv = w_qkv.detach().float().reshape(w_qkv.shape[0], -1)
+    if tuple(w_in.shape) != (PROJ_QKV_C, PROJ_QKV_C) or tuple(w_qkv.shape) != (PROJ_QKV_N, PROJ_QKV_C):
+        raise ValueError(f"sd_amd.proj_qkv_pack: unsupported shapes {tuple(w_in.shape)} / {tuple(w_qkv.shape)}")
+    perm = proj_qkv_perm().to(w_in.device)
+    b_in = torch.zeros(PROJ_QKV_C, device=w_in.device) if b_in is None else b_in.detach().float()
+    b_qkv = torch.zeros(PROJ_QKV_N, device=w_in.device) if b_qkv is None else b_qkv.detach().float().to(w_in.device)
+    return torch.cat([w_in[perm], w_qkv.to(w_in.device)], 0), torch.cat([b_in[perm], b_qkv], 0)
+
+
+def proj_qkv_unpack(w, b):
+    perm = proj_qkv_perm().to(w.device)
+    w_in, b_in = torch.empty_like(w[:PROJ_QKV_C]), torch.empty_like(b[:PROJ_QKV_C])
+    w_in[perm], b_in[perm] = w[:PROJ_QKV_C], b[:PROJ_QKV_C]
+    return w_in, b_in, w[PROJ_QKV_C:], b[PROJ_QKV_C:]
+
+
+def proj_norm_qkv_supported(in_features, features, qkv_features):
+    return bool(lib().sdk_proj_norm_qkv_supported(in_features, features, qkv_features))
+
+
+_CU_COUNT = {}
+
+
+def cu_count(dev):
+    key = torch.device(dev)
+    if key not in _CU_COUNT:
+        _CU_COUNT[key] = torch.cuda.get_device_properties(key).multi_processor_count
+    return _CU_COUNT[key]
+
+
+def proj_qkv_chain_fills(rows, cus):
+    panels = (rows + PROJ_QKV_PANEL - 1) // PROJ_QKV_PANEL
+    last = panels % cus
+    return panels <= cus or last == 0 or 2 * last >= cus
+
+
+class PackedProjQkv:
+
+    def __init__(self, w_in, b_in, w_qkv, device, b_qkv=None):
+        w, b = proj_qkv_pack(w_in, b_in, w_qkv, b_qkv)
+        self.w = w.to(device=device, dtype=torch.float16).contiguous()
+        self.b = b.to(device=device, dtype=torch.float32).contiguous()
+
+
+def proj_norm_qkv(pk: PackedProjQkv, x, norm, gn=None, hw=None, tok=None, qkv=None):
+    _need_cuda(x, "proj_norm_qkv x")
+    M, K = x.shape
+    if K != PROJ_QKV_C or x.stride(-1) != 1:
+        raise ValueError("sd_amd.proj_norm_qkv: x must be [M, 320] with unit column stride")
+    g, bt, eps = norm
+    _need_cuda(g, "proj_norm_qkv gamma", torch.float32)
+    _need_cuda(bt, "proj_norm_qkv beta", torch.float32)
+    if g.numel() != PROJ_QKV_C or bt.numel() != PROJ_QKV_C:
+        raise ValueError("sd_amd.proj_norm_qkv: norm gamma / beta must have 320 elements")
+    if tok is None:
+        tok = torch.empty(M, PROJ_QKV_C, dtype=torch.float16, device=x.device)
+    if qkv is None:
+        qkv = torch.empty(M, PROJ_QKV_N, dtype=torch.float16, device=x.device)
+    _claim(tok)
+    _claim(qkv)
+    a = ProjNormQkvArgs()
+    a.x, a.w, a.bias, a.gamma, a.beta = x.data_ptr(), pk.w.data_ptr(), pk.b.data_ptr(), g.data_ptr(), bt.data_ptr()
+    a.tok, a.qkv = tok.data_ptr(), qkv.data_ptr()
+    a.x_ld, a.tok_ld, a.qkv_ld = x.stride(0), tok.stride(0), qkv.stride(0)
+    a.rows, a.in_features, a.features, a.qkv_features = M, K, tok.shape[1], qkv.shape[1]
+    a.eps = float(eps)
+    if gn is not None:
+        sc, sh = gn
+        _need_cuda(sc, "proj_norm_qkv gn scale", torch.float32)
+        _need_cuda(sh, "proj_norm_qkv gn shift", torch.float32)
+        if hw and (not sc.is_contiguous() or not sh.is_contiguous() or sc.numel() != M // hw * PROJ_QKV_C
+                   or sh.numel() != sc.numel()):
+            raise ValueError("sd_amd.proj_norm_qkv: gn scale / shift must be contiguous fp32 [M / hw, 320]")
+        a.gn_scale, a.gn_shift = sc.data_ptr(), sh.data_ptr()
+    a.hw = int(hw or 0)
+    if PROFILER.active:
+        PROFILER.begin("proj_norm_qkv", None, shape=(M, PROJ_QKV_C + PROJ_QKV_N, K),
+                       nbytes=2 * M * (K + PROJ_QKV_C + PROJ_QKV_N))
+        PROFILER._cur = PROFILER._cur[:2] + (2.0 * M * K * (PROJ_QKV_C + PROJ_QKV_N),) + PROFILER._cur[3:]
+    check(lib().sdk_proj_norm_qkv(C.byref(a), _stream()), "proj_norm_qkv")
+    if PROFILER.active:
+        PROFILER.end()
+    return tok, qkv
+
+
 
 def token_embedding(ids: torch.Tensor, tok: torch.Tensor, pos: torch.Tensor):
     _need_cuda(ids, "token_embedding", torch.int64)
diff --git a/stable-diffusion-from-scratch_amd/packing.py b/stable-diffusion-from-scratch_amd/packing.py
--- a/stable-diffusion-from-scratch_amd/packing.py
+++ b/stable-diffusion-from-scratch_amd/packing.py
@@ -47,6 +47,10 @@
 
 def gn_affine(gn, x):
     return ops.group_norm_affine(x, gn._g, gn._b, gn.eps, gn.num_groups)
+
+
+def gn_scale_shift(gn, x):
+    return ops.group_norm_scale_shift(x, gn._g, gn._b, gn.eps, gn.num_groups)
 
 
 def gn_norm(gn, x, silu=True, pad=0):
```

After: 18.22 images/sec (median of 6 runs). 1.1% higher.
